# ictnlp/StreamSpeech

Measured on AMD Instinct MI355X. Metric: real-time factor (RTFx = audio seconds / wall seconds) + utterances/sec, offline S2ST fr-en, higher is better.
Workload: dtype f32

## Files before the change

### include/streamspeech_hip.h

```cpp
#ifndef STREAMSPEECH_HIP_H
#define STREAMSPEECH_HIP_H

#include <stddef.h>
#include <stdint.h>

#ifdef __cplusplus
extern "C" {
#endif

#define SS_ABI_VERSION 2

typedef struct ss_model ss_model;
typedef struct ss_vocoder ss_vocoder;
typedef struct ss_scratch ss_scratch;
typedef struct ss_stream_pool ss_stream_pool;

typedef struct ss_config {
  int32_t input_feat, conv_channels, conv_kernel;
  int32_t enc_dim, enc_ffn, enc_heads, enc_layers, dw_kernel;
  int32_t src_vocab, tgt_vocab;
  int32_t mt_layers, dec_dim, dec_ffn, dec_heads;
  int32_t t2u_layers, unit_layers, unit_vocab, ctc_upsample;
  int32_t pad, eos, unk;
  int32_t max_rel_pos;
// ... 308 lines not shown
int ss_batch_cmvn(ss_model* m, void* stream, const float* d_in, int64_t rows, float* d_out);
int ss_batch_encoder_forward(ss_model* m, void* stream, int B, const float* d_fbank, const int32_t* h_T,
                             int attn_chunk, int conv_chunk, float* d_enc_out, int32_t* h_Tp);
int ss_batch_ctc_greedy(ss_model* m, void* stream, int head, int B, const float* d_enc_out,
                        const int32_t* h_Tp, int32_t* d_raw, int32_t* d_tokens, int32_t* d_index,
                        int32_t* d_counts);
int ss_batch_ctc_greedy_scored(ss_model* m, void* stream, int head, int B, const float* d_enc_out,
                               const int32_t* h_Tp, int32_t* d_raw, int32_t* d_tokens, int32_t* d_index,
                               int32_t* d_counts, float* d_lprob, int32_t* d_last, float* d_tok_lprob);
typedef struct ss_ctc_align_result {
  double score;
  double viterbi;
  int32_t status;
  int32_t n_tokens;
} ss_ctc_align_result;
#define SS_CTC_ALIGN_MAX_FRAMES 1500
#define SS_CTC_ALIGN_MAX_LABELS 1500
int ss_batch_ctc_align(ss_model* m, void* stream, int head, int B, const float* d_enc_out, const int32_t* h_Tp,
                       const int32_t* h_targets, const int32_t* h_n_targets, ss_ctc_align_result* d_results, int32_t* d_path,
                       int32_t* d_first, int32_t* d_last, float* d_tok_lprob);
int ss_ctc_align_host(const float* h_logits, int ld, int V, int pad, int B, const int32_t* h_T, const int32_t* h_targets,
                      const int32_t* h_n_targets, ss_ctc_align_result* h_results, int32_t* h_path, int32_t* h_first, int32_t* h_last,
                      float* h_tok_lprob, float* h_frame_lprob);
int ss_batch_mt_greedy(ss_model* m, void* stream, int B, const float* d_enc_out, const int32_t* h_Tp,
                       const int32_t* h_max_len, int min_len, int32_t* h_out_tokens, int out_stride,
                       int32_t* h_n_out, float* d_feats, int feat_rows);
int ss_batch_mt_beam(ss_model* m, void* stream, int B, int beam, const float* d_enc_out, const int32_t* h_Tp,
                     const int32_t* h_max_len, int min_len, float unk_penalty, int normalize, int32_t* h_out_tokens,
                     int out_stride, int32_t* h_n_out, float* h_scores, float* h_pos_scores, float* d_feats, int feat_rows);
int ss_batch_mt_continue(ss_model* m, void* stream, int B, const float* d_enc_out, const int32_t* h_Tp, const int32_t* h_prefix,
                         const int32_t* h_n_prefix, const int32_t* h_max_len, int min_len, int32_t* h_out_tokens, int out_stride,
                         int32_t* h_n_out, float* d_feats, int feat_rows, int32_t* h_n_feats);
int ss_batch_mt_continue_plan(int B, const int32_t* h_Tp, const int32_t* h_prefix, const int32_t* h_n_prefix, const int32_t* h_max_len,
                              int min_len, int out_stride, int feat_rows, int max_tgt_pos, int vocab, int eos, int32_t* h_dims,
                              int32_t* h_tables, int64_t tables_cap, int64_t* h_n_tables);
int ss_batch_mt_beam_continue(ss_model* m, void* stream, int B, int beam, const float* d_enc_out, const int32_t* h_Tp,
                              const int32_t* h_prefix, const int32_t* h_n_prefix, const int32_t* h_max_len, int min_len,
                              float unk_penalty, int normalize, int32_t* h_out_tokens, int out_stride, int32_t* h_n_out,
                              float* h_scores, float* h_pos_scores, float* d_feats, int feat_rows);
int ss_batch_mt_beam_continue_plan(int B, int beam, const int32_t* h_Tp, const int32_t* h_prefix, const int32_t* h_n_prefix,
                                   const int32_t* h_max_len, int min_len, int out_stride, int feat_rows, int max_tgt_pos, int vocab,
                                   int eos, int pad, int32_t* h_dims, int32_t* h_tables, int64_t tables_cap, int64_t* h_n_tables);
typedef struct ss_mt_search_opts {
  int32_t size;
  int32_t no_repeat_ngram;
  float len_penalty;
  float temperature;
} ss_mt_search_opts;
int ss_batch_mt_beam_opts(ss_model* m, void* stream, int B, int beam, const float* d_enc_out, const int32_t* h_Tp,
                          const int32_t* h_max_len, int min_len, float unk_penalty, int normalize, int32_t* h_out_tokens,
                          int out_stride, int32_t* h_n_out, float* h_scores, float* h_pos_scores, float* d_feats, int feat_rows,
                          const ss_mt_search_opts* opts);
int ss_batch_mt_beam_continue_opts(ss_model* m, void* stream, int B, int beam, const float* d_enc_out, const int32_t* h_Tp,
                                   const int32_t* h_prefix, const int32_t* h_n_prefix, const int32_t* h_max_len, int min_len,
                                   float unk_penalty, int normalize, int32_t* h_out_tokens, int out_stride, int32_t* h_n_out,
                                   float* h_scores, float* h_pos_scores, float* d_feats, int feat_rows,
                                   const ss_mt_search_opts* opts);
int ss_batch_mt_beam_continue_plan_opts(int B, int beam, const int32_t* h_Tp, const int32_t* h_prefix, const int32_t* h_n_prefix,
                                        const int32_t* h_max_len, int min_len, int out_stride, int feat_rows, int max_tgt_pos,
                                        int vocab, int eos, int pad, int32_t* h_dims, int32_t* h_tables, int64_t tables_cap,
                                        int64_t* h_n_tables, const ss_mt_search_opts* opts);
typedef struct ss_mt_sample_opts {
  int32_t size;
  int32_t topk;
  float topp;
  int32_t reserved;
  uint64_t seed;
} ss_mt_sample_opts;
int ss_batch_mt_sample(ss_model* m, void* stream, int B, int beam, const float* d_enc_out, const int32_t* h_Tp,
                       const int32_t* h_max_len, int min_len, float unk_penalty, int normalize, int32_t* h_out_tokens, int out_stride,
                       int32_t* h_n_out, float* h_scores, float* h_pos_scores, float* d_feats, int feat_rows,
                       const ss_mt_search_opts* opts, const int64_t* h_keys, const ss_mt_sample_opts* sample);
int ss_batch_mt_sample_continue(ss_model* m, void* stream, int B, int beam, const float* d_enc_out, const int32_t* h_Tp,
                                const int32_t* h_prefix, const int32_t* h_n_prefix, const int32_t* h_max_len, int min_len,
                                float unk_penalty, int normalize, int32_t* h_out_tokens, int out_stride, int32_t* h_n_out,
                                float* h_scores, float* h_pos_scores, float* d_feats, int feat_rows, const ss_mt_search_opts* opts,
                                const int64_t* h_keys, const ss_mt_sample_opts* sample);
int ss_batch_fbank_frames(ss_model* m, void* stream, int B, const float* const* h_pcm, const int32_t* h_first, const int32_t* h_n,
                          float pcm_scale, float* const* h_feat);
int ss_batch_fbank_frames_sr(ss_model* m, void* stream, int B, const float* const* h_pcm, const int32_t* h_n_in, const int32_t* h_up,
                             const int32_t* h_down, const float* const* h_taps, const int32_t* h_half_len, const int32_t* h_first,
                             const int32_t* h_n, float pcm_scale, float* const* h_feat);
int ss_fbank_sr_rows(int64_t n_in, int up, int down, int half_len, int32_t* h_n_rows, int32_t* h_n_final);
int ss_batch_t2u_units(ss_model* m, void* stream, int B, const float* d_feats, int feat_rows,
                       const int32_t* h_n, int t2u_causal, int mask_eos, int32_t* d_raw, int32_t* d_tokens,
                       int32_t* d_counts);
int ss_batch_vocoder_forward(ss_vocoder* v, void* stream, int B, const int32_t* d_codes, const int32_t* h_K,
                             int dur_prediction, const int32_t* d_forced_dur, float* d_wav,
                             int64_t wav_capacity, int32_t* d_dur, int64_t* h_wav_start,
                             int64_t* h_n_samples);
int ss_batch_vocoder_forward_spkr(ss_vocoder* v, void* stream, int B, const int32_t* d_codes, const int32_t* h_K,
                                  int dur_prediction, const int32_t* d_forced_dur, float* d_wav,
                                  int64_t wav_capacity, int32_t* d_dur, int64_t* h_wav_start,
                                  int64_t* h_n_samples, const int32_t* h_spkr );
int ss_batch_t2u_units_pad(ss_model* m, void* stream, int B, const float* d_feats, int feat_rows, const int32_t* h_n,
                           const int32_t* h_n_tail_pad, int t2u_causal, int mask_eos, int32_t* d_raw, int32_t* d_tokens,
                           int32_t* d_counts);
int ss_batch_mt_features(ss_model* m, void* stream, int B, const float* d_enc_out, const int32_t* h_Tp, const int32_t* h_tokens,
                         const int32_t* h_n_tokens, const int32_t* h_n_tail_pad, float* d_feats, int feat_rows);
int ss_batch_mt_attention(ss_model* m, void* stream, int B, const float* d_enc_out, const int32_t* h_Tp, const int32_t* h_tokens,
                          const int32_t* h_n_tokens, const int32_t* h_first, float* d_feats, int feat_rows, float* d_attn,
                          int64_t* h_attn_off, int64_t attn_capacity, int32_t* d_peak, float* d_stat);
int ss_batch_mt_score(ss_model* m, void* stream, int U, const float* d_enc_out, const int32_t* h_Tp, int B, const int32_t* h_src,
                      const int32_t* h_tokens, const int32_t* h_n_tokens, float* d_feats, int feat_rows, float* d_stat,
                      int32_t* d_idx);
int ss_batch_vocoder_tail(ss_vocoder* v, void* stream, int B, const int32_t* d_codes, const int32_t* h_K, const int32_t* h_n_new,
                          const int32_t* h_ctx, const int32_t* h_rf, int dur_prediction, float* d_out, int64_t out_capacity,
                          int32_t* h_win_first, int32_t* h_dur, int64_t* h_out_start, int64_t* h_n_out);
int ss_batch_vocoder_tail_spkr(ss_vocoder* v, void* stream, int B, const int32_t* d_codes, const int32_t* h_K, const int32_t* h_n_new,
                               const int32_t* h_ctx, const int32_t* h_rf, int dur_prediction, float* d_out, int64_t out_capacity,
                               int32_t* h_win_first, int32_t* h_dur, int64_t* h_out_start, int64_t* h_n_out,
                               const int32_t* h_spkr );

int ss_batch_unit_spans(ss_model* m, void* stream, int B, const int32_t* d_raw, const int32_t* h_n, const int32_t* h_K,
                        const int32_t* h_dur_first, const int32_t* h_unit0, const int32_t* d_dur, const int32_t* h_dur,
                        int32_t* h_spans, int32_t* h_K_out);
int ss_unit_spans_host(int B, const int32_t* h_raw, const int32_t* h_n, const int32_t* h_K, const int32_t* h_dur_first,
                       const int32_t* h_unit0, const int32_t* h_dur, int up, int blank, int pad, int bos, int eos, int32_t* h_spans,
                       int32_t* h_K_out);

int ss_prof_enable(int cls_mask);
int ss_prof_enable_hi(int cls_mask);
int ss_prof_reset(void);
int ss_prof_read(int cls, double* h_ms_total, double* h_flops_total, int64_t* h_launches,
                 double* h_bytes_total);
int ss_prof_totals(int cls, double* h_flops_total, double* h_bytes_total, int64_t* h_launches);
int ss_prof_read_issued(int cls, double* h_issued_flops_total);
int ss_prof_shape_log(int on);
int ss_prof_shape_dump(char* buf, int cap);
int ss_prof_num_classes(void);
const char* ss_prof_class_name(int cls);

int ss_model_set_pack_invariant(ss_model* m, int on);
int ss_model_get_pack_invariant(ss_model* m);
int ss_debug_canon(int mode);

int ss_debug_last_logits(ss_model* m, void* stream, float* d_out, int64_t cap_floats, int* h_rows, int* h_cols);

int ss_op_ffn_fused(void* stream, const float* dX, int ldx, float* dY, int ldy, const float* ln_g, const float* ln_b,
                    const float* dW1, const float* db1, const float* dW2, const float* db2, float alpha,
                    const float* ln2_g, const float* ln2_b, int M, int D, int F);
int ss_debug_ffn(int grid, int row_tiles_per_wave, int enable);
int ss_debug_rtlin(int grid, int enable);
int ss_debug_rtlin_kb(int uw, int order);
int ss_debug_rtlin_kb_last(int32_t out[4]);
int ss_debug_conv_c64(int enable);
int ss_debug_conv_c256_rows(int rows);
int ss_debug_conv_c32(int enable);
int ss_debug_conv_c16(int enable);
int64_t ss_debug_enc_step_launches(void);
int ss_op_ln_linear(void* stream, const float* dX, int ldx, const float* ln_g, const float* ln_b, const float* dW,
                    const float* dbias, const float* dR, int ldr, float* dC, int ldc, int M, int N, int K, int act, float alpha,
                    int glu);
int ss_op_ln_linear_ex(void* stream, const float* dX, int ldx, const float* ln_g, const float* ln_b, float* ln_out, const float* dW,
                       const float* dbias, const float* dR, int ldr, float* dC, int ldc, int M, int N, int K, int act, float alpha,
                       int glu, int canon);

int ss_debug_force_tile(int bm, int bn, int ks);
int ss_debug_sk_errors(void);
int ss_debug_attention_split(int v);
int ss_debug_attention_q16(int v);
int ss_debug_enc_step_inject_timeout(ss_model* m);
int ss_debug_scratch_audit(ss_scratch* sc, size_t* booked, size_t* held);
int ss_debug_mt_inject_timeout(ss_model* m);

int ss_op_conv_gemm(void* stream, const float* dA, int lda, const float* dW, const float* dbias,
                    const float* dR, int ldr, const float* dR2, int ldr2, float* dC, int ldc,
                    int M, int N, int Cin, int taps, int dil, int stride, int pad, int in_len,
                    int chunk, int in_act, float in_slope, int act, float alpha, float div, int glu);
typedef struct ss_op_conv_args {
  const float* A; const float* W; const float* bias; const float* R; const float* R2; float* C; float* C2;
  int32_t lda, ldc, ldr, ldr2, ldc2;
  int32_t M, N, Cin, taps, dil, stride, pad, in_len, chunk;
  int32_t in_act; float in_slope;
  int32_t act; float act_slope, alpha, div, c2_slope;
  int32_t glu;
  const int32_t* segs; int32_t nseg, max_seg_out;
  int32_t same_rows;
} ss_op_conv_args;
int ss_op_conv_gemm_ex(void* stream, const ss_op_conv_args* a);
int ss_op_conv_gemm_rows(void* stream, const ss_op_conv_args* a, int m_begin, const int32_t* seg_mb, const float* const* seg_A, int canon);
int ss_op_conv_pair(void* stream, const float* dA, int lda, const float* dW1, const float* db1, const float* dW2, const float* db2,
                    float* dC, int ldc, const float* dR2, int ldr2, float div, float* dC2, int ldc2, float c2_slope, int C, int taps,
                    int dil, int M, int in_len, float slope, const int32_t* d_segs, int nseg);
int ss_op_resblock_fused(void* stream, const float* dX, int ldx, const float* const* dW1, const float* const* dB1,
                         const float* const* dW2, const float* const* dB2, const int32_t* dil, float* dY, int ldy, const float* dR2,
                         int ldr2, float div, int C, int taps, int M, float slope, const int32_t* d_segs, int nseg);
int ss_debug_slab(int grid, long long min_rows);
int ss_op_conv_f16(void* stream, const float* dA, const float* dW, const float* dbias, const float* dR, const float* dR2,
                   float* dC, float* dC2, int M, int C, int taps, int dil, int in_act, float in_slope, int act, float div,
                   const int32_t* d_segs, int nseg);
int ss_op_layernorm(void* stream, const float* dx, int ldx, float* dy, int ldy, const float* dg,
                    const float* db, int M, int D, float eps);
int ss_op_attention(void* stream, const float* dQ, int ldq, const float* dK, int ldk, const float* dV,
                    int ldv, float* dO, int ldo, int Tq, int Tk, int H, float scale, int causal,
                    int chunk, const float* dP, int ldp, const float* du, const float* dv);
typedef struct ss_op_attn_args {
  const float* Q; const float* K; const float* V; float* O;
  int32_t ldq, ldk, ldv, ldo;
  int32_t Tq, Tk, H;
  float scale;
  int32_t causal, chunk, q0, k_mask_tail;
  const float* P; int32_t ldp;
  const float* bias_u; const float* bias_v;
  const int32_t* segs; int32_t nseg, max_q, p_tmax;
  const int32_t* seg_tail;
  int32_t no_decode_kernel;
  const int32_t* anc; int32_t anc_ld, anc_slots;
  int32_t use_split;
} ss_op_attn_args;
int ss_op_attention_ex(void* stream, const ss_op_attn_args* a);
typedef struct ss_op_attn_probs_args {
  const float* Q; const float* K;
  int32_t ldq, ldk, H;
  float scale;
  const int32_t* segs; int32_t nseg;
  const int32_t* q_first; const int32_t* row_off; const int64_t* p_off;
  float* P; int32_t* peak; float* stat;
  int32_t max_rows;
} ss_op_attn_probs_args;
int ss_op_attention_probs(void* stream, const ss_op_attn_probs_args* a);
typedef struct ss_op_pool_attn_args {
  const float* Qs; float* cache; float* O;
  int32_t ld, ldo, slot_rows;
  const float* P; int32_t ldp, p_tmax;
  const float* bias_u; const float* bias_v;
  const int32_t* sess; const int32_t* qt_pre;
  int32_t nsess, qtiles, H;
// ... 92 lines not shown
```

### streamspeech_amd/csrc/batch.hip

```cpp
#include <cstring>
#include "model_internal.hpp"
#include "ctc_align.hpp"

extern "C" int ss_batch_fbank_cmvn(ss_model* m, void* stream, int B, const float* d_pcm, const int64_t* h_pcm_start,
                                   const int32_t* h_n_samples, float pcm_scale, float* d_feat, int32_t* h_T) {
  if (!m || B <= 0 || !d_pcm || !d_feat || !h_pcm_start || !h_n_samples || !h_T) return SS_ERR_ARG;
  int64_t rows = 0;
  for (int b = 0; b < B; ++b) {
    if (h_n_samples[b] < 0 || h_pcm_start[b] < 0 || h_pcm_start[b] > (int64_t)0x7fffffff) return SS_ERR_ARG;
    rows += ss_fbank_num_frames(h_n_samples[b]);
  }
  if (rows > (int64_t)0x7fffffff) return SS_ERR_ARG;
  hipStream_t s = (hipStream_t)stream;
  std::vector<int> segs(3 * (size_t)B);
  int row = 0;
  for (int b = 0; b < B; ++b) {
    const int T = ss_fbank_num_frames(h_n_samples[b]);
    h_T[b] = T;
    segs[3 * (size_t)b] = (int)h_pcm_start[b]; segs[3 * (size_t)b + 1] = T; segs[3 * (size_t)b + 2] = row;
    row += T;
  }
  if (row == 0) return SS_OK;
  RET(m->sc->seg_buf.ensure(segs.size() * sizeof(int)));
  const int* dt = (const int*)m->sc->seg_buf.p;
  RET(upload(s, (int*)m->sc->seg_buf.p, segs));
  constexpr int kSlice = 65535;
  for (int b0 = 0; b0 < B; b0 += kSlice) {
    const int nb = std::min(kSlice, B - b0);
    int mx = 0;
    for (int b = b0; b < b0 + nb; ++b) mx = std::max(mx, segs[3 * (size_t)b + 1]);
    RET(launch_fbank_cmvn_batch(d_pcm, pcm_scale, m->fe_window, m->fe_melw, m->fe_mean, m->fe_std, d_feat, dt + 3 * (size_t)b0, nb,
                                mx, s));
  }
  return SS_OK;
}

extern "C" int ss_batch_cmvn(ss_model* m, void* stream, const float* d_in, int64_t rows, float* d_out) {
  if (!m || rows < 0 || (rows > 0 && (!d_in || !d_out))) return SS_ERR_ARG;
  return launch_cmvn_rows(d_in, rows, m->fe_mean, m->fe_std, d_out, (hipStream_t)stream);
}

extern "C" int ss_batch_encoder_forward(ss_model* m, void* stream, int B, const float* d_fbank, const int32_t* h_T,
                                        int attn_chunk, int conv_chunk, float* d_enc_out, int32_t* h_Tp) {
  if (!m || B <= 0) return SS_ERR_ARG;
  SkScope sk_scope(m->sc->skws);
  CanonScope canon_scope(m->pack_invariant ? CANON_SEQ : CANON_NONE);
  const bool canon = m->pack_invariant && !debug_tile_forced();
  hipStream_t s = (hipStream_t)stream;
  const ss_config& c = m->cfg;
  const int d = c.enc_dim, f = c.enc_ffn, k = c.conv_kernel, Ld = c.enc_layers * d;
  std::vector<int> T1(B), T2(B);
  for (int b = 0; b < B; ++b) {
    if (h_T[b] <= 0) return SS_ERR_ARG;
    T1[b] = conv_out_len(h_T[b], k, 2); T2[b] = conv_out_len(T1[b], k, 2);
    if (T2[b] <= 0 || T2[b] > c.max_rel_pos) return SS_ERR_CAPACITY;
    h_Tp[b] = T2[b];
  }
  const Offsets o0 = prefix(h_T, B), o1 = prefix(T1.data(), B), o2 = prefix(T2.data(), B);
  const int M1 = o1.total, M2 = o2.total;
  const int cchunk = conv_chunk_cfg(conv_chunk);
  const int achunk = attn_chunk_cfg(attn_chunk);

  std::vector<int> tab(14 * B);
  int* t0 = tab.data(); int* t1 = t0 + 4 * B; int* ta = t1 + 4 * B; int* tr = ta + 4 * B;
  for (int b = 0; b < B; ++b) {
    t0[4 * b] = o1.off[b]; t0[4 * b + 1] = T1[b]; t0[4 * b + 2] = o0.off[b]; t0[4 * b + 3] = h_T[b];
    t1[4 * b] = o2.off[b]; t1[4 * b + 1] = T2[b]; t1[4 * b + 2] = o1.off[b]; t1[4 * b + 3] = T1[b];
    ta[4 * b] = o2.off[b]; ta[4 * b + 1] = T2[b]; ta[4 * b + 2] = o2.off[b]; ta[4 * b + 3] = T2[b];
    tr[2 * b] = o2.off[b]; tr[2 * b + 1] = T2[b];
  }
  RET(m->sc->seg_buf.ensure(tab.size() * sizeof(int)));
  int* dt = (int*)m->sc->seg_buf.p;
  RET(upload(s, dt, tab));
  const int *d0 = dt, *d1 = dt + 4 * B, *da = dt + 8 * B, *dr = dt + 12 * B;

  const size_t n_h1 = (size_t)M1 * (c.conv_channels / 2), n_x = (size_t)M2 * d, n_f = (size_t)M2 * f,
               n_qkv = (size_t)M2 * 3 * d;
  RET(m->sc->ws.ensure((n_h1 + 3 * n_x + n_f + n_qkv) * sizeof(float)));
  float* h1 = m->sc->ws.f();
  float* x = d_enc_out;
  float* h = h1 + n_h1;
  float* g = h + n_x;
  float* g2 = g + n_x;
  float* ff = g2 + n_x;
  float* qkv = ff + n_f;
  GemmArgs a, b;
  subsampler_args(m, d_fbank, h1, g, a, b);
  a.chunk = cchunk; a.segs = d0; a.nseg = B; a.max_seg_out = o1.mx; a.M = M1; a.in_len = o0.total;
  b.chunk = cchunk; b.segs = d1; b.nseg = B; b.max_seg_out = o2.mx; b.M = M2; b.in_len = M1;
  RET(launch_conv_gemm(a, s));
  RET(launch_conv_gemm(b, s));
  RET(linear(s, g, d, M2, m->enc_linear, d, d, x, d));
  for (int l = 0; l < c.enc_layers; ++l) {
    const EncLayer& e = m->enc[l];
    const bool fuse_ffn = (canon || (disp().ffn_fusion && M2 >= disp().ffn_min_rows)) && ffn_fused_eligible(d, f, ACT_SILU, M2, d, d, canon) &&
                          e.ffn1_w1.b && e.ffn1_w2.b && e.ffn2_w1.b && e.ffn2_w2.b;
    if (canon && !fuse_ffn) return SS_ERR_ARG;
    auto attention = [&] {
      AttnArgs at;
      at.Q = qkv; at.K = qkv + d; at.V = qkv + 2 * d; at.ldq = at.ldk = at.ldv = 3 * d;
      at.O = h; at.ldo = d; at.H = c.enc_heads; at.scale = 0.125f; at.chunk = achunk;
      at.P = m->pos_proj + (size_t)l * d; at.ldp = Ld; at.p_tmax = c.max_rel_pos; at.bias_u = e.u; at.bias_v = e.v;
      at.segs = da; at.nseg = B; at.max_q = o2.mx;
      return launch_attention(at, s);
    };
    auto dwconv = [&] {
      return launch_dwconv_bn_silu(g, d, g2, d, e.dw_wt, c.dw_kernel, e.bn_mean, e.bn_var, e.bn_g, e.bn_b, 1e-5f, o2.mx, d, cchunk, s,
                                   dr, B);
    };
    RET(enc_layer_ex(s, c, e, x, M2, h, ff, qkv, g, g2, fuse_ffn, canon, attention, dwconv));
  }
  return SS_OK;
}

// ... 103 lines not shown
  int Lmax = 0;
  for (int b = 0; b < B; ++b) {
    if (h_Tp[b] <= 0 || h_max_len[b] < 0) return SS_ERR_ARG;
    Lmax = std::max(Lmax, h_max_len[b]);
  }
  const int Lcap = Lmax + 2;
  if (Lcap > feat_rows || Lcap + 2 > c.max_tgt_pos || out_stride < Lmax + 1) return SS_ERR_CAPACITY;
  const Offsets oe = prefix(h_Tp, B);
  RET(m->sc->mt_cross.ensure((size_t)c.mt_layers * oe.total * 2 * D * sizeof(float)));
  RET(mt_cross_kv(m, s, d_enc_out, oe.total));
  RET(m->sc->bmt_self.ensure((size_t)c.mt_layers * B * Lcap * 3 * D * sizeof(float)));
  RET(m->sc->mt_ws.ensure(MtRowsWs::floats(B, D, F, V) * sizeof(float)));
  const MtRowsWs w(m->sc->mt_ws.f(), B, D, F);
  const size_t n_tok = (size_t)(Lcap + 1) * B;
  RET(m->sc->seg_buf.ensure((n_tok + B + 4 * B + (size_t)Lcap * 4 * B) * sizeof(int)));
  int* tok = (int*)m->sc->seg_buf.p;
  int* d_maxlen = tok + n_tok;
  int* d_cross = d_maxlen + B;
  int* d_self = d_cross + 4 * B;
  {
    std::vector<int> t0(B, c.eos), ml(h_max_len, h_max_len + B), cs(4 * B), ss((size_t)Lcap * 4 * B);
    for (int b = 0; b < B; ++b) { cs[4 * b] = b; cs[4 * b + 1] = 1; cs[4 * b + 2] = oe.off[b]; cs[4 * b + 3] = h_Tp[b]; }
    for (int st = 0; st < Lcap; ++st)
      for (int b = 0; b < B; ++b) {
        int* e = &ss[((size_t)st * B + b) * 4];
        e[0] = b; e[1] = 1; e[2] = b * Lcap; e[3] = st + 1;
      }
    RET(upload(s, tok, t0)); RET(upload(s, d_maxlen, ml)); RET(upload(s, d_cross, cs)); RET(upload(s, d_self, ss));
  }
  std::vector<int> host_tok(n_tok, c.pad);
  std::vector<int> eos_at(B, -1);
  int checked = 1;
  int step = 0;
  constexpr int kCheck = 4;
  CanonScope decode_scope(m->pack_invariant ? CANON_SMALLM : CANON_NONE);
  while (true) {
    MtRowsStep a;
    a.rows = B; a.cache_ld = Lcap; a.ci = step; a.tok = tok + (size_t)step * B;
    a.self_segs = d_self + (size_t)step * 4 * B; a.cross_segs = d_cross; a.n_enc = oe.total;
    a.states = d_feats + (size_t)step * D; a.states_ld = feat_rows * D;
    RET(mt_decode_rows(m, s, w, a));
    RET(launch_masked_argmax(w.logits, V, B, V, c.pad, step < min_len ? c.eos : -1, -1, -1, tok + (size_t)(step + 1) * B, s,
                             d_maxlen, step, c.eos));
    ++step;
    const bool last = step > Lmax;
    if (last || step % kCheck == 0) {
      SS_HIP_CHECK(hipMemcpyAsync(host_tok.data() + (size_t)checked * B, tok + (size_t)checked * B,
                                  (size_t)(step + 1 - checked) * B * sizeof(int), hipMemcpyDeviceToHost, s));
      SS_HIP_CHECK(hipStreamSynchronize(s));
      bool all_done = true;
      for (int b = 0; b < B; ++b) {
        for (int r = checked; r <= step && eos_at[b] < 0; ++r)
          if (host_tok[(size_t)r * B + b] == c.eos) eos_at[b] = r;
        if (eos_at[b] < 0) all_done = false;
      }
      checked = step + 1;
      if (all_done || last) break;
    }
  }
  for (int b = 0; b < B; ++b) {
    const int end = eos_at[b] >= 0 ? eos_at[b] : step;
    h_n_out[b] = end;
    for (int r = 1; r <= end; ++r) h_out_tokens[(size_t)b * out_stride + (r - 1)] = host_tok[(size_t)r * B + b];
  }
  return SS_OK;
}

static int batch_t2u(ss_model* m, void* stream, int B, const float* d_feats, int feat_rows, const int32_t* h_n, const int32_t* h_pad,
                     int t2u_causal, int mask_eos, int32_t* d_raw, int32_t* d_tokens, int32_t* d_counts) {
  if (!m || B <= 0 || !h_n) return SS_ERR_ARG;
  SkScope sk_scope(m->sc->skws);
  CanonScope canon_scope(m->pack_invariant ? CANON_SEQ : CANON_NONE);
  hipStream_t s = (hipStream_t)stream;
  const ss_config& c = m->cfg;
  const int D = c.dec_dim, F = c.dec_ffn, V = c.unit_vocab, H = c.dec_heads, up = c.ctc_upsample;
  for (int b = 0; b < B; ++b)
    if (h_n[b] <= 0) return SS_ERR_ARG;
  if (h_pad)
    for (int b = 0; b < B; ++b)
      if (h_pad[b] < 0 || h_pad[b] >= h_n[b]) return SS_ERR_ARG;
  const Offsets on = prefix(h_n, B);
  const int Nn = on.total, U = Nn * up;
  const size_t nx = (size_t)U * D;
  RET(m->sc->ws.ensure((3 * nx + (size_t)U * 3 * D + (size_t)U * F + (size_t)Nn * 2 * D + (size_t)Nn * D +
                    (size_t)U * V + (size_t)U) * sizeof(float)));
  float* x = m->sc->ws.f();
  float* h = x + nx;
  float* q2 = h + nx;
  float* selfbuf = q2 + nx;
  float* ff = selfbuf + (size_t)U * 3 * D;
  float* crosskv = ff + (size_t)U * F;
  float* t2u_out = crosskv + (size_t)Nn * 2 * D;
  float* logits = t2u_out + (size_t)Nn * D;
  int32_t* idx_scratch = reinterpret_cast<int32_t*>(logits + (size_t)U * V);
  std::vector<int> tab(14 * B + Nn + (h_pad ? 3 * B : 0));
  for (int b = 0; b < B; ++b) {
    const int o = on.off[b], n = h_n[b];
    for (int r = 0; r < n; ++r) tab[14 * B + o + r] = b * feat_rows + r;
    int* a = &tab[4 * b]; a[0] = o; a[1] = n; a[2] = o; a[3] = n;
    int* u = &tab[4 * B + 4 * b]; u[0] = o * up; u[1] = n * up; u[2] = o * up; u[3] = n * up;
    int* x2 = &tab[8 * B + 4 * b]; x2[0] = o * up; x2[1] = n * up; x2[2] = o; x2[3] = n;
    tab[12 * B + 2 * b] = o * up; tab[12 * B + 2 * b + 1] = n * up;
    if (h_pad) {
      int* k = &tab[14 * B + Nn];
      k[b] = h_pad[b]; k[B + b] = h_pad[b] * up; k[2 * B + b] = h_pad[b];
    }
  }
  RET(m->sc->seg_buf.ensure(tab.size() * sizeof(int)));
  int* dt = (int*)m->sc->seg_buf.p;
  RET(upload(s, dt, tab));
  const int* tail = h_pad ? dt + 14 * B + Nn : nullptr;
  for (int b = 0; b < B; ++b)
    if (h_n[b] > feat_rows) return SS_ERR_CAPACITY;
  RET(launch_gather_rows(dt + 14 * B, d_feats, D, x, Nn, s, B * feat_rows));
  for (int l = 0; l < c.t2u_layers; ++l) {
    AttnArgs at;
    at.Q = selfbuf; at.ldq = 3 * D; at.K = selfbuf + D; at.V = selfbuf + 2 * D; at.ldk = at.ldv = 3 * D;
    at.O = h; at.ldo = D; at.H = H; at.scale = 1.f; at.causal = t2u_causal ? 1 : 0;
    at.segs = dt; at.nseg = B; at.max_q = on.mx;
    at.no_decode_kernel = m->pack_invariant;
    at.seg_tail = tail;
    RET(dec_layer_ex(s, c, m->t2u[l], x, Nn, selfbuf, 3 * D, at, nullptr, h, q2, ff));
  }
  RET(launch_layernorm(x, D, t2u_out, D, m->t2u_ln.g, m->t2u_ln.b, Nn, D, 1e-5f, s));
  RET(launch_upsample_add_pos(t2u_out, Nn, up, m->unit_pos_row, (float)c.pad, x, D, s));
  for (int l = 0; l < c.unit_layers; ++l) {
    RET(linear(s, t2u_out, D, Nn, m->unit[l].cross_kv, 2 * D, D, crosskv, 2 * D));
    AttnArgs at;
    at.Q = selfbuf; at.ldq = 3 * D; at.K = selfbuf + D; at.V = selfbuf + 2 * D; at.ldk = at.ldv = 3 * D;
    at.O = h; at.ldo = D; at.H = H; at.scale = 1.f; at.causal = 1;
    at.segs = dt + 4 * B; at.nseg = B; at.max_q = on.mx * up; at.no_decode_kernel = m->pack_invariant;
    AttnArgs ac;
    ac.Q = q2; ac.ldq = D; ac.K = crosskv; ac.V = crosskv + D; ac.ldk = ac.ldv = 2 * D;
    ac.O = h; ac.ldo = D; ac.H = H; ac.scale = 1.f; ac.segs = dt + 8 * B; ac.nseg = B; ac.max_q = on.mx * up;
    ac.no_decode_kernel = m->pack_invariant;
    if (tail) { at.seg_tail = tail + B; ac.seg_tail = tail + 2 * B; }
    RET(dec_layer_ex(s, c, m->unit[l], x, U, selfbuf, 3 * D, at, &ac, h, q2, ff));
  }
  RET(launch_layernorm(x, D, h, D, m->unit_ln.g, m->unit_ln.b, U, D, 1e-5f, s));
  RET(linear(s, h, D, U, m->unit_out, V, D, logits, V));
  m->sc->dbg_logits = logits; m->sc->dbg_rows = U; m->sc->dbg_cols = V;
  RET(launch_masked_argmax(logits, V, U, V, c.pad, c.unk, mask_eos ? c.eos : -1, -1, d_raw, s));
  return launch_ctc_collapse(d_raw, 0, V - 1, c.pad, d_tokens, idx_scratch, d_counts, s, dt + 12 * B, B);
}

extern "C" int ss_batch_t2u_units(ss_model* m, void* stream, int B, const float* d_feats, int feat_rows,
                                  const int32_t* h_n, int t2u_causal, int mask_eos, int32_t* d_raw, int32_t* d_tokens,
                                  int32_t* d_counts) {
  return batch_t2u(m, stream, B, d_feats, feat_rows, h_n, nullptr, t2u_causal, mask_eos, d_raw, d_tokens, d_counts);
}

extern "C" int ss_batch_t2u_units_pad(ss_model* m, void* stream, int B, const float* d_feats, int feat_rows, const int32_t* h_n,
                                      const int32_t* h_n_tail_pad, int t2u_causal, int mask_eos, int32_t* d_raw, int32_t* d_tokens,
                                      int32_t* d_counts) {
  if (!h_n_tail_pad) return SS_ERR_ARG;
  return batch_t2u(m, stream, B, d_feats, feat_rows, h_n, h_n_tail_pad, t2u_causal, mask_eos, d_raw, d_tokens, d_counts);
}

struct McPlan {
  int S = 0, Tn = 0, Lcap = 0, Tr = 0, Np = 0, np_max = 0;
  std::vector<int> head;
};
static int mt_continue_plan(int B, const int32_t* h_Tp, const int32_t* h_prefix, const int32_t* h_n_prefix, const int32_t* h_max_len,
                            int min_len, int out_stride, int feat_rows, int max_tgt_pos, int vocab, int eos, McPlan& P) {
  if (B <= 0 || B > 256 || !h_Tp || !h_n_prefix || !h_max_len) return SS_ERR_ARG;
  int S = 0, Tn = 0, Np = 0, np_max = 0;
  for (int b = 0; b < B; ++b) {
    const int st = h_n_prefix[b];
    if (h_Tp[b] <= 0 || st < 0 || h_max_len[b] < st) return SS_ERR_ARG;
    if (st > 0 && !h_prefix) return SS_ERR_ARG;
    S = std::max(S, st);
    Tn = std::max(Tn, h_max_len[b] - st);
    Np += st + 1;
    np_max = std::max(np_max, st + 1);
  }
  {
    int o = 0;
    for (int b = 0; b < B; ++b) {
      for (int i = 0; i < h_n_prefix[b]; ++i)
        if (h_prefix[o + i] < 0 || h_prefix[o + i] >= vocab) return SS_ERR_ARG;
      o += h_n_prefix[b];
    }
  }
  for (int b = 0; b < B; ++b)
    if (h_max_len[b] + 1 > feat_rows || h_max_len[b] - h_n_prefix[b] + 1 > out_stride || h_max_len[b] + 3 > max_tgt_pos)
      return SS_ERR_CAPACITY;
  const int Lcap = S + 1 + Tn, Tr = std::max(Tn, 1);
  const Offsets oe = prefix(h_Tp, B);
  std::vector<int> seg_len(B);
  for (int b = 0; b < B; ++b) seg_len[b] = h_n_prefix[b] + 1;
  const Offsets op = prefix(seg_len.data(), B);
  const size_t np = (size_t)Np;
  P.S = S; P.Tn = Tn; P.Lcap = Lcap; P.Tr = Tr; P.Np = Np; P.np_max = np_max;
  P.head.assign(15 * (size_t)B + (size_t)Tr * 4 * B + 4 * np + B, 0);
  int* ml = P.head.data(); int* mn = ml + B; int* rp = mn + B; int* cs = rp + B; int* ps = cs + 4 * B; int* pc = ps + 4 * B;
  int* ls = pc + 4 * B; int* pt = ls + (size_t)Tr * 4 * B; int* pp = pt + np; int* pk = pp + np; int* pf = pk + np; int* pl = pf + np;
  int o = 0;
  for (int b = 0; b < B; ++b) {
    const int st = h_n_prefix[b], sh = S - st, r0 = op.off[b];
    ml[b] = h_max_len[b] + sh; mn[b] = min_len + sh; rp[b] = -sh;
    cs[4 * b] = b; cs[4 * b + 1] = 1; cs[4 * b + 2] = oe.off[b]; cs[4 * b + 3] = h_Tp[b];
    ps[4 * b] = r0; ps[4 * b + 1] = st + 1; ps[4 * b + 2] = r0; ps[4 * b + 3] = st + 1;
    pc[4 * b] = r0; pc[4 * b + 1] = st + 1; pc[4 * b + 2] = oe.off[b]; pc[4 * b + 3] = h_Tp[b];
    for (int t = 0; t < Tr; ++t) {
      int* e = &ls[((size_t)t * B + b) * 4];
      e[0] = b; e[1] = 1; e[2] = b * Lcap + sh; e[3] = st + 2 + t;
    }
    for (int p = 0; p <= st; ++p) {
      pt[r0 + p] = p == 0 ? eos : h_prefix[o + p - 1];
      pp[r0 + p] = p;
      pk[r0 + p] = b * Lcap + sh + p;
      pf[r0 + p] = b * feat_rows + p;
    }
    pl[b] = r0 + st;
    o += st;
  }
  return SS_OK;
}

// ... 237 lines not shown
  hipStream_t s = (hipStream_t)stream;
  int* dt = (int*)m->sc->seg_buf.p;
  RET(upload(s, dt, tab));
  const int *d_self = dt, *d_cross = dt + 4 * B, *d_tail = dt + 8 * B, *d_tok = dt + 9 * B, *d_pos = d_tok + np, *d_frow = d_pos + np;
  RET(mt_cross_kv(m, s, d_enc_out, oe.total));
  const float* pfo = nullptr;
  RET(mt_prefix_pass(m, s, B, Np, op.mx, oe.total, d_tok, d_pos, d_self, d_cross, d_tail, nullptr, 0, &pfo));
  if (d_feats) RET(launch_scatter_rows(d_frow, pfo, D, d_feats, D, D, Np, B * feat_rows, s));
  if (so) {
    float* logits = m->sc->ws.f() + np * (7 * D + F);
    const int* d_tgt = dt + n_base;
    Lin proj{m->mt_emb, nullptr};
    for (int r0 = 0; r0 < Np; r0 += kMtScoreChunk) {
      const int rows = std::min(kMtScoreChunk, Np - r0);
      RET(linear(s, pfo + (size_t)r0 * D, D, rows, proj, V, D, logits, V));
      RET(launch_mt_token_scores(logits, V, rows, V, d_tgt + r0, so->d_stat + 2 * (size_t)r0, so->d_idx + 2 * (size_t)r0, s));
    }
    return SS_OK;
  }
  if (!ao) return SS_OK;
  AttnProbsArgs ap;
  ap.Q = m->sc->ws.f() + 2 * np * D; ap.ldq = D;
  ap.K = m->sc->mt_cross.f() + (size_t)(c.mt_layers - 1) * oe.total * 2 * D; ap.ldk = 2 * D;
  ap.H = c.dec_heads; ap.scale = 1.f;
  ap.segs = d_cross; ap.nseg = B;
  ap.q_first = dt + n_base; ap.row_off = dt + n_base + B;
  ap.p_off = reinterpret_cast<const long long*>(dt + n_off);
  ap.P = ao->d_attn; ap.peak = ao->d_peak; ap.stat = ao->d_stat; ap.max_rows = max_rows;
  return launch_attention_probs(ap, s);
}

extern "C" int ss_batch_mt_features(ss_model* m, void* stream, int B, const float* d_enc_out, const int32_t* h_Tp,
                                    const int32_t* h_tokens, const int32_t* h_n_tokens, const int32_t* h_n_tail_pad, float* d_feats,
                                    int feat_rows) {
  if (!h_n_tail_pad || !d_feats) return SS_ERR_ARG;
  return batch_mt_features(m, stream, B, d_enc_out, h_Tp, h_tokens, h_n_tokens, h_n_tail_pad, d_feats, feat_rows, nullptr);
}

extern "C" int ss_batch_mt_attention(ss_model* m, void* stream, int B, const float* d_enc_out, const int32_t* h_Tp,
                                     const int32_t* h_tokens, const int32_t* h_n_tokens, const int32_t* h_first, float* d_feats,
                                     int feat_rows, float* d_attn, int64_t* h_attn_off, int64_t attn_capacity, int32_t* d_peak,
                                     float* d_stat) {
  if (!d_peak || !d_stat || attn_capacity < 0) return SS_ERR_ARG;
  MtAttnOut ao;
  ao.h_first = h_first; ao.d_attn = d_attn; ao.h_attn_off = h_attn_off; ao.attn_capacity = attn_capacity;
  ao.d_peak = d_peak; ao.d_stat = d_stat;
  return batch_mt_features(m, stream, B, d_enc_out, h_Tp, h_tokens, h_n_tokens, nullptr, d_feats, feat_rows, &ao);
}

extern "C" int ss_batch_mt_score(ss_model* m, void* stream, int U, const float* d_enc_out, const int32_t* h_Tp, int B,
                                 const int32_t* h_src, const int32_t* h_tokens, const int32_t* h_n_tokens, float* d_feats,
                                 int feat_rows, float* d_stat, int32_t* d_idx) {
  if (!d_stat || !d_idx) return SS_ERR_ARG;
  MtScoreOut so;
  so.U = U; so.h_src = h_src; so.d_stat = d_stat; so.d_idx = d_idx;
  return batch_mt_features(m, stream, B, d_enc_out, h_Tp, h_tokens, h_n_tokens, nullptr, d_feats, feat_rows, nullptr, &so);
}

extern "C" int ss_batch_fbank_frames(ss_model* m, void* stream, int B, const float* const* h_pcm, const int32_t* h_first,
                                     const int32_t* h_n, float pcm_scale, float* const* h_feat) {
  if (!m || B <= 0 || B > 65535 || !h_pcm || !h_first || !h_n || !h_feat) return SS_ERR_ARG;
  constexpr int kShift = 160;
  int mx = 0;
  for (int b = 0; b < B; ++b) {
    if (h_first[b] < 0 || h_n[b] < 0 || ((int64_t)h_first[b] + (int64_t)h_n[b]) * kShift > (int64_t)0x7fffffff) return SS_ERR_ARG;
    if (h_n[b] > 0 && (!h_pcm[b] || !h_feat[b])) return SS_ERR_ARG;
    mx = std::max(mx, h_n[b]);
  }
  if (mx == 0) return SS_OK;
  hipStream_t s = (hipStream_t)stream;
  const size_t n_seg = (3 * (size_t)B + 1) & ~(size_t)1;
  std::vector<int> tab(n_seg + 4 * (size_t)B, 0);
  int64_t* ptrs = reinterpret_cast<int64_t*>(tab.data() + n_seg);
  for (int b = 0; b < B; ++b) {
    tab[3 * b] = h_first[b] * kShift; tab[3 * b + 1] = h_n[b]; tab[3 * b + 2] = 0;
    ptrs[b] = (int64_t)(uintptr_t)h_pcm[b];
    ptrs[B + b] = (int64_t)(uintptr_t)h_feat[b];
  }
  RET(m->sc->seg_buf.ensure(tab.size() * sizeof(int)));
  int* dt = (int*)m->sc->seg_buf.p;
  RET(upload(s, dt, tab));
  const float* const* d_pcm = reinterpret_cast<const float* const*>(dt + n_seg);
  float* const* d_feat = reinterpret_cast<float* const*>(dt + n_seg + 2 * (size_t)B);
  return launch_fbank_cmvn_ptrs(d_pcm, d_feat, pcm_scale, m->fe_window, m->fe_melw, m->fe_mean, m->fe_std, dt, B, mx, s);
}

extern "C" int ss_batch_fbank_frames_sr(ss_model* m, void* stream, int B, const float* const* h_pcm, const int32_t* h_n_in,
                                        const int32_t* h_up, const int32_t* h_down, const float* const* h_taps,
                                        const int32_t* h_half_len, const int32_t* h_first, const int32_t* h_n, float pcm_scale,
                                        float* const* h_feat) {
  if (!m || B <= 0 || B > 65535 || !h_pcm || !h_n_in || !h_up || !h_down || !h_taps || !h_half_len || !h_first || !h_n || !h_feat)
    return SS_ERR_ARG;
  static_assert(sizeof(FbankSrSeg) % sizeof(int) == 0, "the segment table is uploaded as ints");
  constexpr size_t kSegInts = sizeof(FbankSrSeg) / sizeof(int);
  std::vector<int> tab(kSegInts * (size_t)B, 0);
  int mx = 0, max_taps = 0;
  for (int b = 0; b < B; ++b) {
    if (h_first[b] < 0 || h_n[b] < 0) return SS_ERR_ARG;
    FbankSrSeg sg{};
    if (h_n[b] > 0) {
      int rows = 0;
      RET(fbank_sr_rows(h_n_in[b], h_up[b], h_down[b], h_half_len[b], &rows, nullptr));
      if ((int64_t)h_first[b] + (int64_t)h_n[b] > (int64_t)rows) return SS_ERR_ARG;
      const bool pass = h_up[b] == h_down[b];
      if (!h_pcm[b] || !h_feat[b] || (!pass && !h_taps[b])) return SS_ERR_ARG;
      sg.pcm = h_pcm[b]; sg.taps = h_taps[b]; sg.feat = h_feat[b];
      sg.n_in = h_n_in[b]; sg.up = h_up[b]; sg.down = h_down[b]; sg.half = h_half_len[b]; sg.first = h_first[b]; sg.n_rows = h_n[b];
      mx = std::max(mx, h_n[b]);
      if (!pass) max_taps = std::max(max_taps, 2 * h_half_len[b] + 1);
    }
    std::memcpy(tab.data() + kSegInts * (size_t)b, &sg, sizeof(sg));
  }
  if (mx == 0) return SS_OK;
  hipStream_t s = (hipStream_t)stream;
  RET(m->sc->seg_buf.ensure(tab.size() * sizeof(int)));
  int* dt = (int*)m->sc->seg_buf.p;
  RET(upload(s, dt, tab));
  return launch_fbank_cmvn_sr(reinterpret_cast<const FbankSrSeg*>(dt), B, mx, max_taps, pcm_scale, m->fe_window, m->fe_melw,
                              m->fe_mean, m->fe_std, s);
}

extern "C" int ss_fbank_sr_rows(int64_t n_in, int up, int down, int half_len, int32_t* h_n_rows, int32_t* h_n_final) {
  int rows = 0, fin = 0;
  RET(fbank_sr_rows(n_in, up, down, half_len, &rows, &fin));
  if (h_n_rows) *h_n_rows = rows;
  if (h_n_final) *h_n_final = fin;
  return SS_OK;
}
```

### streamspeech_amd/csrc/debug_ops.hip

```cpp
#include "model_internal.hpp"
#include "ctc_align.hpp"

static int op_bind_wino(GemmArgs& a, void* stream) {
  static thread_local std::map<hipStream_t, DevBuf> wino_tmps;
  DevBuf& wino_tmp = wino_tmps[(hipStream_t)stream];
  const int N = a.N, Cin = a.Cin, taps = a.taps;
  if ((conv_c64w_enabled() && N == 64 && Cin == 64 && taps >= 3 && conv_c64_eligible(a)) ||
      (conv_c128w_enabled() && N == 128 && Cin == 128 && taps >= 3 && a.same_rows && !a.glu) ||
      (conv_c256w_enabled() && N == 256 && Cin == 256 && taps >= 3 && a.same_rows && !a.glu) ||
      (conv_c32w_enabled() && N == 32 && Cin == 32 && taps >= 3 && conv_c32_eligible(a))) {
    RET(wino_tmp.ensure((size_t)N * ((taps + 2) / 3) * 4 * N * sizeof(float)));
    RET(launch_wino_pack(a.W, wino_tmp.f(), N, taps, (hipStream_t)stream));
    a.Wwino = wino_tmp.f();
  }
  return SS_OK;
}

extern "C" int ss_op_conv_gemm(void* stream, const float* dA, int lda, const float* dW, const float* dbias,
                               const float* dR, int ldr, const float* dR2, int ldr2, float* dC, int ldc, int M,
                               int N, int Cin, int taps, int dil, int stride, int pad, int in_len, int chunk,
                               int in_act, float in_slope, int act, float alpha, float div, int glu) {
  GemmArgs a;
  a.A = dA; a.lda = lda; a.W = dW; a.bias = dbias; a.R = dR; a.ldr = ldr; a.R2 = dR2; a.ldr2 = ldr2; a.C = dC; a.ldc = ldc;
  a.M = M; a.N = N; a.Cin = Cin; a.taps = taps; a.dil = dil; a.stride = stride; a.pad = pad; a.in_len = in_len;
// ... 69 lines not shown

extern "C" int ss_debug_last_logits(ss_model* m, void* stream, float* d_out, int64_t cap_floats, int* h_rows, int* h_cols) {
  if (!m || !h_rows || !h_cols) return SS_ERR_ARG;
  *h_rows = m->sc->dbg_rows; *h_cols = m->sc->dbg_cols;
  if (!d_out) return SS_OK;
  if (!m->sc->dbg_logits || cap_floats < (int64_t)m->sc->dbg_rows * m->sc->dbg_cols) return SS_ERR_CAPACITY;
  SS_HIP_CHECK(hipMemcpyAsync(d_out, m->sc->dbg_logits, (size_t)m->sc->dbg_rows * m->sc->dbg_cols * sizeof(float), hipMemcpyDeviceToDevice,
                              (hipStream_t)stream));
  return SS_OK;
}

extern "C" int ss_op_ffn_fused(void* stream, const float* dX, int ldx, float* dY, int ldy, const float* ln_g, const float* ln_b,
                               const float* dW1, const float* db1, const float* dW2, const float* db2, float alpha,
                               const float* ln2_g, const float* ln2_b, int M, int D, int F) {
  return launch_ffn_fused(dX, ldx, dY, ldy, ln_g, ln_b, dW1, db1, dW2, db2, alpha, ln2_g, ln2_b, M, D, F, (hipStream_t)stream,
                          canon_mode() == CANON_SEQ);
}
extern "C" int ss_debug_canon(int mode) {
  if (mode < 0 || mode > 2) return SS_ERR_ARG;
  canon_debug_set(mode);
  return SS_OK;
}
extern "C" int ss_op_ln_linear(void* stream, const float* dX, int ldx, const float* ln_g, const float* ln_b, const float* dW,
                               const float* dbias, const float* dR, int ldr, float* dC, int ldc, int M, int N, int K, int act,
                               float alpha, int glu) {
  GemmArgs a;
  a.A = dX; a.lda = ldx; a.W = dW; a.bias = dbias; a.R = dR; a.ldr = ldr; a.C = dC; a.ldc = ldc;
  a.M = M; a.N = N; a.Cin = K; a.in_len = M; a.act = act; a.alpha = alpha; a.glu = glu; a.same_rows = 1;
  a.ln_g = ln_g; a.ln_b = ln_b;
  return launch_conv_gemm(a, (hipStream_t)stream);
}
extern "C" int ss_op_ln_linear_ex(void* stream, const float* dX, int ldx, const float* ln_g, const float* ln_b, float* ln_out,
                                  const float* dW, const float* dbias, const float* dR, int ldr, float* dC, int ldc, int M, int N, int K,
                                  int act, float alpha, int glu, int canon) {
  if (canon < 0 || canon > 2 || (ln_g == nullptr) != (ln_b == nullptr) || (ln_out && !ln_g)) return SS_ERR_ARG;
  GemmArgs a;
  a.A = dX; a.lda = ldx; a.W = dW; a.bias = dbias; a.R = dR; a.ldr = ldr; a.C = dC; a.ldc = ldc;
  a.M = M; a.N = N; a.Cin = K; a.in_len = M; a.act = act; a.alpha = alpha; a.glu = glu; a.same_rows = 1;
  a.ln_g = ln_g; a.ln_b = ln_b; a.ln_out = ln_out; a.canon = canon;
  return launch_conv_gemm(a, (hipStream_t)stream);
}
extern "C" int ss_debug_conv_c64(int enable) {
  if (enable == 4 || enable == 5) { conv_c64w_debug(enable == 5); return SS_OK; }
  if (enable == 6 || enable == 7) { conv_c128w_debug(enable == 7); return SS_OK; }
  if (enable == 8 || enable == 9) { conv_c256w_debug(enable == 9); return SS_OK; }
  conv_c64_debug(enable);
  return SS_OK;
}
extern "C" int ss_debug_conv_c256_rows(int rows) { return conv_c256w_rows_debug(rows); }
extern "C" int ss_debug_conv_c32(int enable) {
  if (enable == 4 || enable == 5) { conv_c32w_debug(enable == 5); return SS_OK; }
  conv_c32_debug(enable);
  return SS_OK;
}
extern "C" int ss_debug_conv_c16(int enable) { conv_c16_debug(enable); return SS_OK; }
extern "C" int64_t ss_debug_enc_step_launches(void) { return (int64_t)enc_step_launch_count(); }
extern "C" int ss_debug_scratch_audit(ss_scratch* sc, size_t* booked, size_t* held) {
  if (!sc || !booked || !held) return SS_ERR_ARG;
  size_t sum = 0;
  bool foreign = false;
  for (DevBuf* b : sc->all()) {
    sum += b->bytes;
    if (b->acct != &sc->acct) foreign = true;
  }
  *booked = sc->acct.used;
  *held = sum;
  return foreign ? SS_ERR_ARG : SS_OK;
}
extern "C" int ss_debug_rtlin(int grid, int enable) {
  if (grid < 0) return SS_ERR_ARG;
  rtlin_debug(grid, enable);
  return SS_OK;
}
extern "C" int ss_debug_rtlin_kb(int uw, int order) {
  if (!(uw == 0 || uw == 1 || uw == 2 || uw == 4) || order < -1 || order > 2) return SS_ERR_ARG;
  rtlin_kb_debug(uw, order);
  return SS_OK;
}
extern "C" int ss_debug_rtlin_kb_last(int32_t out[4]) {
  if (!out) return SS_ERR_ARG;
  int v[4];
  rtlin_kb_last(v);
  for (int i = 0; i < 4; ++i) out[i] = v[i];
  return SS_OK;
}
extern "C" int ss_debug_ffn(int grid, int row_tiles_per_wave, int enable) {
  if (grid < 0 || row_tiles_per_wave < -1 || row_tiles_per_wave > 4) return SS_ERR_ARG;
  ffn_fused_debug_grid(grid);
  ffn_fused_debug_rows(row_tiles_per_wave);
  if (enable >= 0) dispatch_edit([enable](Dispatch& d) { d.ffn_fusion = enable ? 1 : 0; });
  return SS_OK;
}

extern "C" int ss_op_layernorm(void* stream, const float* dx, int ldx, float* dy, int ldy, const float* dg,
                               const float* db, int M, int D, float eps) {
  return launch_layernorm(dx, ldx, dy, ldy, dg, db, M, D, eps, (hipStream_t)stream);
}

extern "C" int ss_op_masked_argmax(void* stream, const float* logits, int ld, int M, int N, int mask0, int mask1, int mask2, int force,
                                   int32_t* ids, const int32_t* row_max_len, int step, int force_id, const int32_t* row_min_len,
                                   int ban_id) {
  return launch_masked_argmax(logits, ld, M, N, mask0, mask1, mask2, force, ids, (hipStream_t)stream, row_max_len, step, force_id,
                              row_min_len, ban_id);
}
extern "C" int ss_op_ctc_collapse(void* stream, const int32_t* raw, int T, int blank, int pad, int32_t* tokens, int32_t* index,
                                  int32_t* count, const int32_t* segs, int nseg) {
  return launch_ctc_collapse(raw, T, blank, pad, tokens, index, count, (hipStream_t)stream, segs, nseg);
}
extern "C" int ss_op_masked_argmax_lprob(void* stream, const float* logits, int ld, int M, int N, int mask0, int mask1, int mask2,
                                         int32_t* ids, float* lprob) {
  return launch_masked_argmax_lprob(logits, ld, M, N, mask0, mask1, mask2, ids, lprob, (hipStream_t)stream);
}
static int g_mt_score_form = 0;
extern "C" int ss_debug_mt_score_form(int v) { g_mt_score_form = v ? 1 : 0; return SS_OK; }
extern "C" int ss_op_mt_token_scores(void* stream, const float* d_logits, int ld, int rows, int V, const int32_t* d_target,
                                     float* d_stat, int32_t* d_idx) {
  return launch_mt_token_scores(d_logits, ld, rows, V, d_target, d_stat, d_idx, (hipStream_t)stream, g_mt_score_form);
}
extern "C" int ss_op_ctc_collapse_spans(void* stream, const int32_t* raw, const float* lprob, int T, int blank, int pad, int32_t* tokens,
                                        int32_t* index, int32_t* last, float* tok_lprob, int32_t* count, const int32_t* segs, int nseg) {
  return launch_ctc_collapse_spans(raw, lprob, T, blank, pad, tokens, index, last, tok_lprob, count, (hipStream_t)stream, segs, nseg);
}
extern "C" int ss_op_ctc_align(void* stream, const float* d_logits, int ld, int V, int pad, int B, const int32_t* h_T,
                               const int32_t* h_targets, const int32_t* h_n_targets, ss_ctc_align_result* d_results, int32_t* d_path,
                               int32_t* d_first, int32_t* d_last, float* d_tok_lprob, float* d_frame_lprob) {
  if (!d_logits || ld < V || !d_results) return SS_ERR_ARG;
  CtcAlignPlan plan;
  RET(ctc_align_plan(V, pad, B, h_T, h_targets, h_n_targets, plan));
  if (plan.labels > 0 && (!d_first || !d_last || !d_tok_lprob)) return SS_ERR_ARG;
  static thread_local std::map<hipStream_t, std::pair<DevBuf, DevBuf>> tmps;
  auto& tmp = tmps[(hipStream_t)stream];
  RET(tmp.first.ensure(ctc_align_table_bytes(plan)));
  RET(tmp.second.ensure(plan.work_bytes()));
  return launch_ctc_align(d_logits, ld, V, plan, h_targets, tmp.first.p, tmp.second.p, d_results, d_path, d_first, d_last, d_tok_lprob,
                          d_frame_lprob, (hipStream_t)stream);
}
extern "C" int ss_op_dur_predict(void* stream, const float* logdur, const int32_t* forced, int K, int32_t* dur, int32_t* cum,
                                 const int32_t* segs, int nseg) {
  return launch_dur_predict(logdur, forced, K, dur, cum, (hipStream_t)stream, segs, nseg);
}
extern "C" int ss_op_repeat_rows(void* stream, const float* emb, const int32_t* cum, int K, int D, float* out, int F,
                                 const int32_t* segs, int nseg) {
  return launch_repeat_rows(emb, cum, K, D, out, F, (hipStream_t)stream, segs, nseg);
}
extern "C" int ss_op_embed_tokens(void* stream, const int32_t* tok, const float* emb, const float* pos_table, float scale, int pos0,
                                  float* out, int n, int D, int pos_stride, int pad_id, int vocab) {
  return launch_embed_tokens(tok, emb, pos_table, scale, pos0, out, n, D, (hipStream_t)stream, pos_stride, pad_id, vocab);
}
extern "C" int ss_op_embed_tokens_rows(void* stream, const int32_t* tok, const float* emb, const float* pos_table, int pos_rows,
                                       float scale, int pos0, const int32_t* row_pos, float* out, int n, int D, int pad_id, int vocab) {
  return launch_embed_tokens_rows(tok, emb, pos_table, pos_rows, scale, pos0, row_pos, out, n, D, (hipStream_t)stream, pad_id, vocab);
}
extern "C" int ss_op_upsample_add_pos(void* stream, const float* src, int n, int up, const float* pos_row, float pad_value, float* out,
                                      int D) {
  return launch_upsample_add_pos(src, n, up, pos_row, pad_value, out, D, (hipStream_t)stream);
}
extern "C" int ss_op_gather_rows(void* stream, const int32_t* idx, const float* table, int D, float* out, int n, int rows) {
  return launch_gather_rows(idx, table, D, out, n, (hipStream_t)stream, rows);
}
extern "C" int ss_op_scatter_rows(void* stream, const int32_t* dst_row, const float* src, int lds, float* dst, int ldd, int D, int n,
                                  int dst_rows) {
  return launch_scatter_rows(dst_row, src, lds, dst, ldd, D, n, dst_rows, (hipStream_t)stream);
}
extern "C" int ss_op_conv_post_tanh(void* stream, const float* x, int T, int C, const float* w, const float* bias, float slope,
                                    float* wav, const int32_t* segs, int nseg) {
  return launch_conv_post_tanh(x, T, C, w, bias, slope, wav, (hipStream_t)stream, segs, nseg);
// ... 117 lines not shown
```

### streamspeech_amd/csrc/dispatch.hip

```cpp
#include "gemm.hpp"

#include <atomic>
#include <cstdlib>
#include <map>
#include <mutex>
#include <utility>
#include <vector>

namespace ss {

namespace {
std::mutex g_disp_mu;
std::atomic<unsigned> g_disp_gen{1};
Dispatch env_defaults() {
  Dispatch d;
  auto I = [](const char* k, int dflt) { const char* e = getenv(k); return e ? atoi(e) : dflt; };
  auto L = [](const char* k, long long dflt) { const char* e = getenv(k); return e ? atoll(e) : dflt; };
  d.attn_split = I("SS_ATTN_NO_SPLIT", 0) ? -1 : 0; d.attn_q16 = I("SS_ATTN_Q16", d.attn_q16);
  d.c16_off = I("SS_NO_CONV_C16", 0) ? 1 : 0; d.c32_off = I("SS_NO_CONV_C32", 0) ? 1 : 0; d.c64_off = I("SS_NO_CONV_C64", 0) ? 1 : 0;
  d.c16_min_rows = L("SS_CONV_C16_MIN_ROWS", d.c16_min_rows); d.c32_min_rows = L("SS_CONV_C32_MIN_ROWS", d.c32_min_rows);
  d.c64_min_rows = L("SS_CONV_C64_MIN_ROWS", d.c64_min_rows);
  d.c64w_on = I("SS_CONV_C64_WINOGRAD", 1); d.c128w_on = I("SS_CONV_C128_WINOGRAD", 1); d.c256w_on = I("SS_CONV_C256_WINOGRAD", 1);
  d.c32w_on = I("SS_CONV_C32_WINOGRAD", 1); d.c64w_min_k = I("SS_CONV_C64_WINOGRAD_MIN_K", 3);
  d.c128w_min_rows = L("SS_CONV_C128_MIN_ROWS", d.c128w_min_rows); d.c256w_min_rows = L("SS_CONV_C256_MIN_ROWS", d.c256w_min_rows);
  if (const int r = I("SS_CONV_C256_ROWS", d.c256w_rows); r == 128 || r == 256) d.c256w_rows = r;
  if (getenv("SS_FFN_WM")) { d.ffn_wm = I("SS_FFN_WM", 3); d.ffn_wm_forced = 1; d.ffn_wm_env = d.ffn_wm; }
  d.ffn_fusion = I("SS_NO_FFN_FUSION", 0) ? 0 : 1; d.ffn_min_rows = I("SS_FFN_MIN_ROWS", d.ffn_min_rows);
  if (getenv("SS_SK_MIN_GFLOP")) d.sk_min_flops = 1e9 * atof(getenv("SS_SK_MIN_GFLOP"));
  d.no_resblock_fusion = I("SS_NO_RESBLOCK_FUSION", 0); d.no_pair_fusion = I("SS_NO_PAIR_FUSION", 0);
  d.rt_off = I("SS_NO_RTLIN", 0) ? 1 : 0; d.rt_min_rows = I("SS_RTLIN_MIN_ROWS", d.rt_min_rows); d.rt_min_units = L("SS_RTLIN_MIN_UNITS", d.rt_min_units);
  d.rt_kb_min_units = L("SS_RTLIN_KB_MIN_UNITS", d.rt_kb_min_units); d.rt_kb_uw = I("SS_RTLIN_KB_UW", d.rt_kb_uw); d.rt_kb_xmap = I("SS_RTLIN_KB_XMAP", d.rt_kb_xmap);
  d.smallm_max_rows = I("SS_SMALLM_MAX_ROWS", d.smallm_max_rows); d.sk_min_units = L("SS_SK_MIN_UNITS", d.sk_min_units);
  d.no_sk2 = I("SS_NO_SK2", 0) ? 1 : 0; d.sk2_min_k64 = I("SS_SK2_MINK64", d.sk2_min_k64); d.sk2_spare_cus = I("SS_SK2_SPARE_CUS", 0);
  d.rt_wg_per_cu = I("SS_RTLIN_WG_PER_CU", 0); d.c32_min_k = I("SS_CONV_C32_MIN_K", d.c32_min_k); d.c16_min_k = I("SS_CONV_C16_MIN_K", d.c16_min_k);
  return d;
}
Dispatch& process_settings() { static Dispatch d = env_defaults(); return d; }
thread_local const Dispatch* t_disp = nullptr;
thread_local CtxDispatch t_disp_own;
}
void dispatch_edit(const std::function<void(Dispatch&)>& fn) {
  std::lock_guard<std::mutex> lk(g_disp_mu);
  fn(process_settings());
  g_disp_gen.fetch_add(1, std::memory_order_release);
}
void slab_debug(int grid, long long min_rows) {
  const Dispatch dflt = env_defaults();
  dispatch_edit([=](Dispatch& d) {
    d.slab_grid_cap = grid > 0 ? grid : 0;
    const bool set = min_rows >= 0;
    d.c16_min_rows = set ? min_rows : dflt.c16_min_rows; d.c32_min_rows = set ? min_rows : dflt.c32_min_rows;
    d.c64_min_rows = set ? min_rows : dflt.c64_min_rows;
    d.c128w_min_rows = set ? min_rows : dflt.c128w_min_rows; d.c256w_min_rows = set ? min_rows : dflt.c256w_min_rows;
  });
}
int conv_c256w_rows_debug(int rows) {
  if (rows != 0 && rows != 128 && rows != 256) return SS_ERR_ARG;
  const int dflt = env_defaults().c256w_rows;
  dispatch_edit([=](Dispatch& d) { d.c256w_rows = rows ? rows : dflt; });
  return SS_OK;
}
const Dispatch* CtxDispatch::refresh() {
  const unsigned now = g_disp_gen.load(std::memory_order_acquire);
  if (gen != now) {
    std::lock_guard<std::mutex> lk(g_disp_mu);
    d = process_settings();
    gen = g_disp_gen.load(std::memory_order_relaxed);
  }
  return &d;
}
const Dispatch& disp() { return t_disp ? *t_disp : *t_disp_own.refresh(); }
DispatchScope::DispatchScope(const Dispatch* d) : prev(t_disp) { t_disp = d; }
DispatchScope::~DispatchScope() { t_disp = prev; }

void debug_force_tile(int bm, int bn, int ks) {
  dispatch_edit([=](Dispatch& d) { d.force_bm = bm; d.force_bn = bn; d.force_ks = ks; d.sk_groups = (bm == 1 && bn == 8); });
}
bool debug_tile_forced() { return disp().force_bm != 0; }

static thread_local int t_canon = CANON_NONE;
CanonScope::CanonScope(int mode) : prev(t_canon) { t_canon = mode; }
CanonScope::~CanonScope() { t_canon = prev; }
int canon_mode() { return t_canon; }
void canon_debug_set(int mode) { t_canon = mode; }

constexpr size_t SKW_SYNC_BYTES = (16 + 1024) * sizeof(unsigned) + 256;
static std::mutex g_skw_mu;
static std::vector<SkWorkspace*> g_skw_live;
static std::map<std::pair<int, hipStream_t>, SkWorkspace*> g_skw_fallback;
static thread_local SkWorkspace* t_skw = nullptr;

SkWorkspace* sk_workspace_new() {
  SkWorkspace* w = new SkWorkspace();
  std::lock_guard<std::mutex> lk(g_skw_mu);
  g_skw_live.push_back(w);
  return w;
}
void sk_workspace_free(SkWorkspace* w) {
  if (!w) return;
  {
    std::lock_guard<std::mutex> lk(g_skw_mu);
    for (size_t i = 0; i < g_skw_live.size(); ++i)
      if (g_skw_live[i] == w) { g_skw_live.erase(g_skw_live.begin() + i); break; }
  }
  if (w->ws) (void)hipFree(w->ws);
  if (w->sync1) (void)hipFree(w->sync1);
  if (w->sync2) (void)hipFree(w->sync2);
  if (w->sync3) (void)hipFree(w->sync3);
  if (w->dbg) (void)hipFree(w->dbg);
  delete w;
}
SkScope::SkScope(SkWorkspace* w) : prev(t_skw), prev_disp(t_disp) { t_skw = w; t_disp = w ? w->disp.refresh() : nullptr; }
SkScope::~SkScope() { t_skw = prev; t_disp = prev_disp; }

int sk_workspace_acquire(hipStream_t stream, SkWorkspace** out) {
  *out = nullptr;
  int dev = 0;
// ... 58 lines not shown
```

### streamspeech_amd/csrc/dispatch.hpp

```cpp
#pragma once
#include <functional>

namespace ss {

struct Dispatch {
  int attn_no_mfma = 0;
  int attn_q16 = 1;
  int attn_split = 0;
  int c16_off = 0, c32_off = 0, c64_off = 0;
  long long c16_min_rows = 131072, c32_min_rows = 65536, c64_min_rows = 32768;
  int c64w_on = 1, c128w_on = 1, c256w_on = 1, c32w_on = 1;
  int c64w_min_k = 3;
  long long c128w_min_rows = 65536, c256w_min_rows = 32768;
  int c256w_rows = 128;
  int c32_min_k = 7, c16_min_k = 11;
  int slab_grid_cap = 0;
  int sk_groups = 0;
  int sk2_spare_cus = 0;
  int ffn_force_g = 0;
  int ffn_wm = 3, ffn_wm_forced = 0;
  int ffn_wm_env = 0;
  int ffn_fusion = 1;
  int ffn_min_rows = 1000;
  int force_bm = 0, force_bn = 0, force_ks = 0;
  double sk_min_flops = 4e9;
  int smallm_max_rows = 192;
  long long sk_min_units = 12 * 512;
  int no_sk2 = 0;
  int sk2_min_k64 = 192;
  int no_resblock_fusion = 0, no_pair_fusion = 0;
  int rt_off = 0, rt_min_rows = 193, rt_force_g = 0;
  long long rt_min_units = 4000;
  int rt_wg_per_cu = 0;
  long long rt_kb_min_units = 256;
  int rt_kb_xmap = 1;
  int rt_kb_uw = 0;
  int rt_kb_order = 1;
};

const Dispatch& disp();
void dispatch_edit(const std::function<void(Dispatch&)>& fn);

struct CtxDispatch {
  Dispatch d;
  unsigned gen = 0xffffffffu;
  const Dispatch* refresh();
};
struct DispatchScope {
  explicit DispatchScope(const Dispatch* d);
  ~DispatchScope();
  const Dispatch* prev;
};

}
```

### streamspeech_amd/csrc/elementwise.hip

```cpp
#include "elementwise.hpp"

namespace ss {

template <int PER_LANE>
__global__ __launch_bounds__(256) void layernorm_kernel(const float* __restrict__ x, int ldx, float* y,
                                                        int ldy, const float* __restrict__ gamma,
                                                        const float* __restrict__ beta, int M, float eps) {
  constexpr int D = PER_LANE * 64;
  const int lane = threadIdx.x & 63;
  const int row = blockIdx.x * 4 + (threadIdx.x >> 6);
  if (row >= M) return;
  const float* xr = x + (size_t)row * ldx;
  float v[PER_LANE];
  float s = 0.f;
#pragma unroll
  for (int i = 0; i < PER_LANE; ++i) { v[i] = xr[lane + 64 * i]; s += v[i]; }
  const float mean = wave_sum(s) / (float)D;
  float q = 0.f;
#pragma unroll
  for (int i = 0; i < PER_LANE; ++i) { const float d = v[i] - mean; q += d * d; }
  const float rstd = 1.0f / sqrtf(wave_sum(q) / (float)D + eps);
  float* yr = y + (size_t)row * ldy;
#pragma unroll
  for (int i = 0; i < PER_LANE; ++i) {
// ... 62 lines not shown
  const float mean = bn_mean[c], rstd = 1.0f / sqrtf(bn_var[c] + bn_eps), gam = bn_gamma[c], bet = bn_beta[c];
  constexpr int NR = DW_TT / 4, NV = NR + DW_KMAX - 1;
  float sv[NV];
#pragma unroll
  for (int i = 0; i < NV; ++i) sv[i] = slab[(rg * NR + i) * DW_TC + cl];
#pragma unroll
  for (int u = 0; u < NR; ++u) {
    const int t = t0 + rg * NR + u;
    int lim = T;
    if (chunk > 0) { const int cl_end = (t / chunk + 1) * chunk; if (cl_end < lim) lim = cl_end; }
    const int jmax = min(K, lim - (t - half));
    float acc = 0.f;
#pragma unroll
    for (int j = 0; j < DW_KMAX; ++j) {
      const float a2 = fmaf(w[j], sv[u + j], acc);
      acc = (j < jmax) ? a2 : acc;
    }
    const float v = (acc - mean) * rstd * gam + bet;
    if (t < T) y[(size_t)t * ldy + c] = v / (1.0f + expf(-v));
  }
}

int launch_dwconv_bn_silu(const float* x, int ldx, float* y, int ldy, const float* wt, int K,
                          const float* bn_mean, const float* bn_var, const float* bn_gamma,
                          const float* bn_beta, float bn_eps, int T, int C, int chunk, hipStream_t stream,
                          const int* segs, int nseg, int t_begin) {
  if (T - t_begin <= 0) return SS_OK;
  if (K > DW_KMAX || (K & 1) == 0 || t_begin < 0) return SS_ERR_ARG;
  dim3 grid(cdiv(C, DW_TC), cdiv(T - t_begin, DW_TT), nseg > 0 ? nseg : 1);
  hipLaunchKernelGGL(dwconv_bn_silu_kernel, grid, dim3(256), 0, stream, x, ldx, y, ldy, wt, K, bn_mean,
                     bn_var, bn_gamma, bn_beta, bn_eps, T, C, chunk, nseg > 0 ? segs : nullptr, t_begin);
  SS_LAUNCH_CHECK();
  return SS_OK;
}

__global__ void embed_tokens_kernel(const int* __restrict__ tok, const float* __restrict__ emb,
                                    const float* __restrict__ pos_table, float scale, int pos0, float* out,
                                    int n, int D, int pos_stride, int pad_id, int vocab, const int* __restrict__ row_pos,
                                    int pos_rows) {
  const int i = blockIdx.y;
  const int c = blockIdx.x * 256 + threadIdx.x;
  if (c >= D) return;
  int tk = tok[i];
  if ((unsigned)tk >= (unsigned)vocab) tk = 0;
  int pos = (tk == pad_id) ? pad_id : pos0 + (row_pos ? row_pos[i] : i * pos_stride);
  if (row_pos && (unsigned)pos >= (unsigned)pos_rows) pos = pos_rows - 1;
  out[(size_t)i * D + c] = scale * emb[(size_t)tk * D + c] + pos_table[(size_t)pos * D + c];
}

int launch_embed_tokens(const int* tok, const float* emb, const float* pos_table, float scale, int pos0,
                        float* out, int n, int D, hipStream_t stream, int pos_stride, int pad_id, int vocab) {
  if (n <= 0) return SS_OK;
  hipLaunchKernelGGL(embed_tokens_kernel, dim3(cdiv(D, 256), n), dim3(256), 0, stream, tok, emb, pos_table,
                     scale, pos0, out, n, D, pos_stride, pad_id, vocab, (const int*)nullptr, 0);
  SS_LAUNCH_CHECK();
  return SS_OK;
}

int launch_embed_tokens_rows(const int* tok, const float* emb, const float* pos_table, int pos_rows, float scale, int pos0,
                             const int* row_pos, float* out, int n, int D, hipStream_t stream, int pad_id, int vocab) {
  if (n <= 0) return SS_OK;
  if (pos_rows <= 0) return SS_ERR_ARG;
  hipLaunchKernelGGL(embed_tokens_kernel, dim3(cdiv(D, 256), n), dim3(256), 0, stream, tok, emb, pos_table,
                     scale, pos0, out, n, D, 0, pad_id, vocab, row_pos, pos_rows);
  SS_LAUNCH_CHECK();
  return SS_OK;
}

__global__ void upsample_add_pos_kernel(const float* __restrict__ src, int up, const float* __restrict__ pos_row,
                                        float pad_value, float* out, int D) {
  const int u = blockIdx.y;
  const int c = blockIdx.x * 256 + threadIdx.x;
  if (c >= D) return;
  const float* s = src + (size_t)(u / up) * D;
  const float add = (s[0] != pad_value) ? pos_row[c] : 0.f;
  out[(size_t)u * D + c] = s[c] + add;
}

int launch_upsample_add_pos(const float* src, int n, int up, const float* pos_row, float pad_value,
                            float* out, int D, hipStream_t stream) {
  if (n <= 0) return SS_OK;
  hipLaunchKernelGGL(upsample_add_pos_kernel, dim3(cdiv(D, 256), n * up), dim3(256), 0, stream, src, up,
                     pos_row, pad_value, out, D);
  SS_LAUNCH_CHECK();
  return SS_OK;
}

__global__ void gather_rows_kernel(const int* __restrict__ idx, const float* __restrict__ table, int D,
                                   float* out, int rows) {
  const int i = blockIdx.y;
  const int c = blockIdx.x * 256 + threadIdx.x;
  if (c >= D) return;
  int r = idx[i];
  if ((unsigned)r >= (unsigned)rows) r = 0;
  out[(size_t)i * D + c] = table[(size_t)r * D + c];
}

int launch_gather_rows(const int* idx, const float* table, int D, float* out, int n, hipStream_t stream, int rows) {
  if (n <= 0) return SS_OK;
  hipLaunchKernelGGL(gather_rows_kernel, dim3(cdiv(D, 256), n), dim3(256), 0, stream, idx, table, D, out, rows);
  SS_LAUNCH_CHECK();
  return SS_OK;
}

__global__ void scatter_rows_kernel(const int* __restrict__ dst_row, const float* __restrict__ src, int lds, float* dst, int ldd,
                                    int D, int dst_rows) {
  const int i = blockIdx.y;
  const int c = blockIdx.x * 256 + threadIdx.x;
  const int r = dst_row[i];
  if (c >= D || (unsigned)r >= (unsigned)dst_rows) return;
  dst[(size_t)r * ldd + c] = src[(size_t)i * lds + c];
}

int launch_scatter_rows(const int* dst_row, const float* src, int lds, float* dst, int ldd, int D, int n, int dst_rows,
                        hipStream_t stream) {
  if (n <= 0) return SS_OK;
  hipLaunchKernelGGL(scatter_rows_kernel, dim3(cdiv(D, 256), n), dim3(256), 0, stream, dst_row, src, lds, dst, ldd, D, dst_rows);
  SS_LAUNCH_CHECK();
  return SS_OK;
}

__global__ __launch_bounds__(256) void masked_argmax_kernel(const float* __restrict__ logits, int ld, int M, int N,
                                                            int mask0, int mask1, int mask2, int force, int* ids,
                                                            const int* __restrict__ row_max_len, int step, int force_id,
                                                            const int* __restrict__ row_min_len, int ban_id) {
  __shared__ float sb[4];
  __shared__ int si[4];
  const int t = threadIdx.x, lane = t & 63, wave = t >> 6;
  const int row = blockIdx.x;
  if (row_max_len && step >= row_max_len[row]) force = force_id;
  if (row_min_len && step < row_min_len[row]) mask1 = ban_id;
  if (force >= 0) { if (t == 0) ids[row] = force; return; }
  const float* r = logits + (size_t)row * ld;
  float best = -INFINITY;
  int bi = 0x7fffffff;
  for (int n = t; n < N; n += 256) {
    if (n == mask0 || n == mask1 || n == mask2) continue;
    float v = r[n];
    if (v != v) v = -INFINITY;
    if (bi == 0x7fffffff || v > best) { best = v; bi = n; }
  }
#pragma unroll
  for (int o = 32; o > 0; o >>= 1) {
    const float ob = __shfl_xor(best, o, 64);
    const int oi = __shfl_xor(bi, o, 64);
    if (oi != 0x7fffffff && (bi == 0x7fffffff || ob > best || (ob == best && oi < bi))) { best = ob; bi = oi; }
  }
  if (lane == 0) { sb[wave] = best; si[wave] = bi; }
  __syncthreads();
  if (t == 0) {
    for (int w = 1; w < 4; ++w) {
      const float ob = sb[w]; const int oi = si[w];
      if (oi != 0x7fffffff && (bi == 0x7fffffff || ob > best || (ob == best && oi < bi))) { best = ob; bi = oi; }
    }
    ids[row] = bi;
  }
}

int launch_masked_argmax(const float* logits, int ld, int M, int N, int mask0, int mask1, int mask2,
                         int force, int* ids, hipStream_t stream, const int* row_max_len, int step, int force_id,
                         const int* row_min_len, int ban_id) {
  if (M <= 0) return SS_OK;
  hipLaunchKernelGGL(masked_argmax_kernel, dim3(M), dim3(256), 0, stream, logits, ld, M, N, mask0,
                     mask1, mask2, force, ids, row_max_len, step, force_id, row_min_len, ban_id);
  SS_LAUNCH_CHECK();
  return SS_OK;
// ... 300 lines not shown
```

### streamspeech_amd/csrc/elementwise.hpp

```cpp
#pragma once
#include "common.hpp"

struct ss_ctc_align_result;

namespace ss {

int launch_layernorm(const float* x, int ldx, float* y, int ldy, const float* gamma, const float* beta,
                     int M, int D, float eps, hipStream_t stream);

int launch_dwconv_bn_silu(const float* x, int ldx, float* y, int ldy, const float* wt, int K,
                          const float* bn_mean, const float* bn_var, const float* bn_gamma,
                          const float* bn_beta, float bn_eps, int T, int C, int chunk, hipStream_t stream,
                          const int* segs = nullptr, int nseg = 0,
                          int t_begin = 0);

int launch_embed_tokens(const int* tok, const float* emb, const float* pos_table, float scale, int pos0,
                        float* out, int n, int D, hipStream_t stream, int pos_stride, int pad_id, int vocab);
int launch_embed_tokens_rows(const int* tok, const float* emb, const float* pos_table, int pos_rows, float scale, int pos0,
                             const int* row_pos, float* out, int n, int D, hipStream_t stream, int pad_id, int vocab);

int launch_upsample_add_pos(const float* src, int n, int up, const float* pos_row, float pad_value,
                            float* out, int D, hipStream_t stream);

int launch_masked_argmax(const float* logits, int ld, int M, int N, int mask0, int mask1, int mask2,
                         int force, int* ids, hipStream_t stream, const int* row_max_len = nullptr, int step = 0,
                         int force_id = -1,
                         const int* row_min_len = nullptr, int ban_id = -1);

int launch_log_softmax(const float* logits, int ld, int M, int N, int mask0, int mask1, int as_probs, float* out, int ldo,
                       hipStream_t stream);
int launch_row_max_logprob(const float* logits, int ld, int M, int N, int mask0, int mask1, int mask2, float* out,
                           hipStream_t stream);

int launch_ctc_collapse(const int* raw, int T, int blank, int pad, int* tokens, int* index, int* count,
                        hipStream_t stream, const int* segs = nullptr, int nseg = 0);

int launch_masked_argmax_lprob(const float* logits, int ld, int M, int N, int mask0, int mask1, int mask2, int* ids, float* lprob,
                               hipStream_t stream);
int launch_ctc_collapse_spans(const int* raw, const float* lprob, int T, int blank, int pad, int* tokens, int* index, int* last,
                              float* tok_lprob, int* count, hipStream_t stream, const int* segs = nullptr, int nseg = 0);

constexpr int MT_SCORE_MAX_ROWS = 16777215;
constexpr int MT_SCORE_MAX_REG_N = 8192;
int launch_mt_token_scores(const float* logits, int ld, int M, int N, const int* target, float* stat, int* idx, hipStream_t stream,
                           int form = 0);

struct CtcAlignPlan;
size_t ctc_align_table_bytes(const CtcAlignPlan& p);
int launch_ctc_align(const float* logits, int ld, int V, const CtcAlignPlan& p, const int32_t* h_targets, void* d_table, void* d_work,
                     ss_ctc_align_result* results, int* path, int* first, int* last, float* tok_lprob, float* frame_lprob,
                     hipStream_t stream);

int launch_gather_rows(const int* idx, const float* table, int D, float* out, int n, hipStream_t stream, int rows);
int launch_scatter_rows(const int* dst_row, const float* src, int lds, float* dst, int ldd, int D, int n, int dst_rows,
                        hipStream_t stream);

int launch_dur_predict(const float* logdur, const int* forced, int K, int* dur, int* cum, hipStream_t stream,
                       const int* segs = nullptr, int nseg = 0);

int launch_repeat_rows(const float* emb, const int* cum, int K, int D, float* out, int F, hipStream_t stream,
                       const int* segs = nullptr, int nseg = 0);

int launch_conv_post_tanh(const float* x, int T, int C, const float* w, const float* bias, float slope,
                          float* wav, hipStream_t stream, const int* segs = nullptr, int nseg = 0);
int launch_conv_post_tanh_crop(const float* x, int C, const float* w, const float* bias, float slope, float* wav, const int* segs,
                               int nseg, int max_keep, hipStream_t stream);

int launch_spkr_pre_add(const float* x, float* y, int ld, int C0, const float* table, const int* spkr, int spkr0, const int* segs,
                        int nseg, int max_seg_out, int M, int act, float slope, hipStream_t stream);

}
```

### streamspeech_amd/csrc/fbank.hip

```cpp
#include "fbank.hpp"

namespace ss {

constexpr int WIN = 400, SHIFT = 160, NFFT = 512, NBIN = 257, NMEL = 80;

__device__ __forceinline__ void fbank_row(const float v0, const float v1, const float pcm_scale,
                                          const float* __restrict__ window,
                                          const float* __restrict__ melw,
                                          const float* __restrict__ cmvn_mean, const float* __restrict__ cmvn_std,
                                          float* __restrict__ feat_row) {
  __shared__ float re[NFFT], im[NFFT];
  __shared__ float tw_c[NFFT / 2], tw_s[NFFT / 2];
  __shared__ float red[4];
  const int t = threadIdx.x, lane = t & 63, wave = t >> 6;
  const float x0 = v0 * pcm_scale;
  const float x1 = (t + 256 < WIN) ? v1 * pcm_scale : 0.f;
  float s = wave_sum(x0 + x1);
  if (lane == 0) red[wave] = s;
  {
    float sn, cs;
    sincospif(-2.0f * (float)t / (float)NFFT, &sn, &cs);
    tw_c[t] = cs; tw_s[t] = sn;
  }
  __syncthreads();
  const float mean = (red[0] + red[1] + red[2] + red[3]) / (float)WIN;
  re[t] = x0 - mean;
  re[t + 256] = (t + 256 < WIN) ? (x1 - mean) : 0.f;
  __syncthreads();
  float y0, y1 = 0.f;
  {
    const float prev0 = re[t > 0 ? t - 1 : 0];
    y0 = (re[t] - 0.97f * prev0) * window[t];
    if (t + 256 < WIN) y1 = (re[t + 256] - 0.97f * re[t + 255]) * window[t + 256];
  }
  __syncthreads();
  re[__brev((unsigned)t) >> 23] = y0;
  re[__brev((unsigned)(t + 256)) >> 23] = y1;
  im[t] = 0.f; im[t + 256] = 0.f;
  __syncthreads();
#pragma unroll
  for (int stg = 0; stg < 9; ++stg) {
    const int half = 1 << stg;
    const int grp = t >> stg, pos = t & (half - 1);
    const int i0 = (grp << (stg + 1)) + pos, i1 = i0 + half;
    const int tk = pos << (8 - stg);
    const float c = tw_c[tk], sn = tw_s[tk];
    const float br = re[i1] * c - im[i1] * sn;
    const float bi = re[i1] * sn + im[i1] * c;
    const float ar = re[i0], ai = im[i0];
    __syncthreads();
    re[i0] = ar + br; im[i0] = ai + bi;
    re[i1] = ar - br; im[i1] = ai - bi;
    __syncthreads();
  }
  const float p0 = re[t] * re[t] + im[t] * im[t];
  const float p256 = (t == 0) ? (re[256] * re[256] + im[256] * im[256]) : 0.f;
  __syncthreads();
  re[t] = p0;
  if (t == 0) re[256] = p256;
  __syncthreads();
  if (t < NMEL) {
    const float* w = melw + t * NBIN;
    float e = 0.f;
    for (int i = 0; i < NBIN; ++i) e = fmaf(w[i], re[i], e);
    const float lg = logf(fmaxf(e, 1.1920928955078125e-07f));
    feat_row[t] = (lg - cmvn_mean[t]) / cmvn_std[t];
  }
}

__global__ __launch_bounds__(256) void fbank_cmvn_kernel(const float* __restrict__ pcm, float pcm_scale,
                                                         const float* __restrict__ window,
                                                         const float* __restrict__ melw,
                                                         const float* __restrict__ cmvn_mean,
                                                         const float* __restrict__ cmvn_std, float* feat,
                                                         const int* __restrict__ segs,
                                                         const float* const* __restrict__ pcm_ptrs,
                                                         float* const* __restrict__ feat_ptrs) {
  const int t = threadIdx.x;
  const int frame = blockIdx.x;
  if (segs) {
    const int* sg = segs + 3 * blockIdx.y;
    if (frame >= sg[1]) return;
    if (pcm_ptrs) { pcm = pcm_ptrs[blockIdx.y]; feat = feat_ptrs[blockIdx.y]; }
    pcm += sg[0]; feat += (size_t)sg[2] * NMEL;
  }
  const float* src = pcm + (size_t)frame * SHIFT;
  fbank_row(src[t], (t + 256 < WIN) ? src[t + 256] : 0.f, pcm_scale, window, melw, cmvn_mean, cmvn_std, feat + (size_t)frame * NMEL);
}

int launch_fbank_cmvn(const float* pcm, int n_samples, float pcm_scale, const float* window,
                      const float* melw, const float* cmvn_mean, const float* cmvn_std, float* feat,
                      int* n_frames, hipStream_t stream) {
  const int T = n_samples < WIN ? 0 : 1 + (n_samples - WIN) / SHIFT;
  if (n_frames) *n_frames = T;
  if (T == 0) return SS_OK;
  hipLaunchKernelGGL(fbank_cmvn_kernel, dim3(T), dim3(256), 0, stream, pcm, pcm_scale, window, melw,
                     cmvn_mean, cmvn_std, feat, (const int*)nullptr, (const float* const*)nullptr, (float* const*)nullptr);
  SS_LAUNCH_CHECK();
  return SS_OK;
}

int launch_fbank_cmvn_batch(const float* pcm, float pcm_scale, const float* window, const float* melw,
                            const float* cmvn_mean, const float* cmvn_std, float* feat, const int* segs, int nseg,
                            int max_frames, hipStream_t stream) {
  if (nseg <= 0 || max_frames <= 0) return SS_OK;
  hipLaunchKernelGGL(fbank_cmvn_kernel, dim3(max_frames, nseg), dim3(256), 0, stream, pcm, pcm_scale, window, melw,
                     cmvn_mean, cmvn_std, feat, segs, (const float* const*)nullptr, (float* const*)nullptr);
  SS_LAUNCH_CHECK();
  return SS_OK;
}

__global__ __launch_bounds__(256) void cmvn_rows_kernel(const float* in, const float* __restrict__ cmvn_mean,
                                                        const float* __restrict__ cmvn_std, float* out, long long n) {
  const long long i = (long long)blockIdx.x * 256 + threadIdx.x;
  if (i >= n) return;
  const int t = (int)(i % NMEL);
  const float lg = in[i];
  out[i] = (lg - cmvn_mean[t]) / cmvn_std[t];
}

int launch_cmvn_rows(const float* in, long long rows, const float* cmvn_mean, const float* cmvn_std, float* out, hipStream_t stream) {
  if (rows <= 0) return SS_OK;
  const long long n = rows * NMEL, blocks = (n + 255) / 256;
  if (blocks > 0x7fffffffLL) return SS_ERR_ARG;
  hipLaunchKernelGGL(cmvn_rows_kernel, dim3((unsigned)blocks), dim3(256), 0, stream, in, cmvn_mean, cmvn_std, out, n);
  SS_LAUNCH_CHECK();
  return SS_OK;
}

int launch_fbank_cmvn_ptrs(const float* const* pcm_ptrs, float* const* feat_ptrs, float pcm_scale, const float* window,
                           const float* melw, const float* cmvn_mean, const float* cmvn_std, const int* segs, int nseg,
                           int max_frames, hipStream_t stream) {
  if (nseg <= 0 || max_frames <= 0) return SS_OK;
  hipLaunchKernelGGL(fbank_cmvn_kernel, dim3(max_frames, nseg), dim3(256), 0, stream, (const float*)nullptr, pcm_scale, window, melw,
                     cmvn_mean, cmvn_std, (float*)nullptr, segs, pcm_ptrs, feat_ptrs);
  SS_LAUNCH_CHECK();
  return SS_OK;
}

__global__ __launch_bounds__(256) void resample_kernel(const float* __restrict__ x, long long n_in, int up, int down,
                                                       const float* __restrict__ h, int half, float* __restrict__ y,
                                                       long long n_out) {
  extern __shared__ float hs[];
  const int ntaps = 2 * half + 1;
  for (int i = threadIdx.x; i < ntaps; i += 256) hs[i] = h[i];
  __syncthreads();
  const long long k = (long long)blockIdx.x * 256 + threadIdx.x;
  if (k >= n_out) return;
  y[k] = resample_sample(x, n_in, up, down, hs, half, k);
}

int launch_resample(const float* x, long long n_in, int up, int down, const float* taps, int half_len, float* y,
                    long long n_out, hipStream_t stream) {
  if (n_in <= 0 || n_out <= 0) return SS_OK;
  if (up <= 0 || down <= 0 || half_len < 0) return SS_ERR_ARG;
  const size_t lds = (size_t)(2 * half_len + 1) * sizeof(float);
  if (lds > 64 * 1024) return SS_ERR_ARG;
  hipLaunchKernelGGL(resample_kernel, dim3((unsigned)((n_out + 255) / 256)), dim3(256), lds, stream, x, n_in, up, down,
                     taps, half_len, y, n_out);
  SS_LAUNCH_CHECK();
  return SS_OK;
}

constexpr size_t FBANK_ROW_LDS = (2 * NFFT + 2 * (NFFT / 2) + 4) * sizeof(float);
constexpr size_t WG_LDS = 64 * 1024;
constexpr int FBANK_SR_MAX_HALF = (int)(((WG_LDS - FBANK_ROW_LDS) / sizeof(float) - 1) / 2);

__global__ __launch_bounds__(256) void fbank_cmvn_sr_kernel(const FbankSrSeg* __restrict__ segs, float pcm_scale,
                                                            const float* __restrict__ window, const float* __restrict__ melw,
                                                            const float* __restrict__ cmvn_mean,
                                                            const float* __restrict__ cmvn_std) {
  extern __shared__ float hs[];
  const FbankSrSeg sg = segs[blockIdx.y];
  if ((int)blockIdx.x >= sg.n_rows) return;
  const int t = threadIdx.x;
  const long long k0 = (long long)(sg.first + (int)blockIdx.x) * SHIFT + t;
  float v0, v1 = 0.f;
  if (sg.up == sg.down) {
    v0 = sg.pcm[k0];
    if (t + 256 < WIN) v1 = sg.pcm[k0 + 256];
  } else {
    const int ntaps = 2 * sg.half + 1;
    for (int i = t; i < ntaps; i += 256) hs[i] = sg.taps[i];
    __syncthreads();
    v0 = resample_sample(sg.pcm, sg.n_in, sg.up, sg.down, hs, sg.half, k0);
    if (t + 256 < WIN) v1 = resample_sample(sg.pcm, sg.n_in, sg.up, sg.down, hs, sg.half, k0 + 256);
  }
  fbank_row(v0, v1, pcm_scale, window, melw, cmvn_mean, cmvn_std, sg.feat + (size_t)blockIdx.x * NMEL);
}

int fbank_sr_rows(long long n_in, int up, int down, int half_len, int* n_rows, int* n_final) {
  if (n_in < 0 || up < 1 || down < 1 || half_len < 0) return SS_ERR_ARG;
  if (half_len > FBANK_SR_MAX_HALF) return SS_ERR_ARG;
  if (n_in > (long long)0x7fffffff || n_in * up > (long long)0x7fffffff * down) return SS_ERR_ARG;
  const long long n16 = (n_in * up + down - 1) / down;
  const long long rows = n16 < WIN ? 0 : 1 + (n16 - WIN) / SHIFT;
  const long long top = n_in * up - 1 - half_len;
  long long fin = 0;
  if (top >= 0) {
    const long long kmax = top / down;
    if (kmax >= WIN - 1) fin = 1 + (kmax - (WIN - 1)) / SHIFT;
  }
  if (fin > rows) fin = rows;
  if (n_rows) *n_rows = (int)rows;
  if (n_final) *n_final = (int)fin;
  return SS_OK;
}

int launch_fbank_cmvn_sr(const FbankSrSeg* segs, int nseg, int max_rows, int max_taps, float pcm_scale, const float* window,
                         const float* melw, const float* cmvn_mean, const float* cmvn_std, hipStream_t stream) {
  if (nseg <= 0 || max_rows <= 0) return SS_OK;
  if (max_taps < 0 || max_taps > 2 * FBANK_SR_MAX_HALF + 1) return SS_ERR_ARG;
  const size_t lds = (size_t)max_taps * sizeof(float);
  hipLaunchKernelGGL(fbank_cmvn_sr_kernel, dim3(max_rows, nseg), dim3(256), lds, stream, segs, pcm_scale, window, melw, cmvn_mean,
                     cmvn_std);
  SS_LAUNCH_CHECK();
  return SS_OK;
}

}
```

### streamspeech_amd/csrc/fbank.hpp

```cpp
#pragma once
#include <math.h>

#include "common.hpp"

namespace ss {

int launch_fbank_cmvn(const float* pcm, int n_samples, float pcm_scale, const float* window,
                      const float* melw, const float* cmvn_mean, const float* cmvn_std, float* feat,
                      int* n_frames, hipStream_t stream);

int launch_fbank_cmvn_batch(const float* pcm, float pcm_scale, const float* window, const float* melw,
                            const float* cmvn_mean, const float* cmvn_std, float* feat, const int* segs, int nseg,
                            int max_frames, hipStream_t stream);

int launch_fbank_cmvn_ptrs(const float* const* pcm_ptrs, float* const* feat_ptrs, float pcm_scale, const float* window,
                           const float* melw, const float* cmvn_mean, const float* cmvn_std, const int* segs, int nseg,
                           int max_frames, hipStream_t stream);

int launch_cmvn_rows(const float* in, long long rows, const float* cmvn_mean, const float* cmvn_std, float* out, hipStream_t stream);

int launch_resample(const float* x, long long n_in, int up, int down, const float* taps, int half_len, float* y,
                    long long n_out, hipStream_t stream);

template <class X>
__host__ __device__ __forceinline__ float resample_sample(X x, long long n_in, int up, int down, const float* hs, int half,
                                                          long long k) {
  const long long c = k * down;
  long long m_lo = c - half;
  m_lo = m_lo <= 0 ? 0 : (m_lo + up - 1) / up;
  long long m_hi = (c + half) / up;
  if (m_hi > n_in - 1) m_hi = n_in - 1;
  float acc = 0.f;
  for (long long m = m_lo; m <= m_hi; ++m) acc = fmaf(x[m], hs[half + (int)(c - m * up)], acc);
  return acc;
}

struct FbankSrSeg {
  const float* pcm;
  const float* taps;
  float* feat;
  int n_in, up, down, half, first, n_rows;
};

int fbank_sr_rows(long long n_in, int up, int down, int half_len, int* n_rows, int* n_final);

int launch_fbank_cmvn_sr(const FbankSrSeg* segs, int nseg, int max_rows, int max_taps, float pcm_scale, const float* window,
                         const float* melw, const float* cmvn_mean, const float* cmvn_std, hipStream_t stream);

}
```

### streamspeech_amd/csrc/model.hip

```cpp
#include "model_internal.hpp"

static int load_dec_layers(ss_model* m, std::vector<DecLayer>& v, const std::string& pfx, int n, int D, int F,
                           int kv_in, bool cross) {
  WeightTable& w = m->wt;
  v.resize(n);
  for (int l = 0; l < n; ++l) {
    const std::string p = pfx + ".L" + std::to_string(l) + ".";
    DecLayer& d = v[l];
    d.has_cross = cross;
    d.self_ln = {w.get(p + "self.ln.g", D), w.get(p + "self.ln.b", D)};
    d.self_qkv = {w.get(p + "self.qkv.w", 3LL * D * D), w.get(p + "self.qkv.b", 3LL * D)};
    d.self_out = {w.get(p + "self.out.w", (int64_t)D * D), w.get(p + "self.out.b", D)};
    if (cross) {
      d.cross_ln = {w.get(p + "cross.ln.g", D), w.get(p + "cross.ln.b", D)};
      d.cross_q = {w.get(p + "cross.q.w", (int64_t)D * D), w.get(p + "cross.q.b", D)};
      d.cross_kv = {w.get(p + "cross.kv.w", 2LL * D * kv_in), w.get(p + "cross.kv.b", 2LL * D)};
      d.cross_out = {w.get(p + "cross.out.w", (int64_t)D * D), w.get(p + "cross.out.b", D)};
    }
    d.ffn_ln = {w.get(p + "ffn.ln.g", D), w.get(p + "ffn.ln.b", D)};
    d.fc1 = {w.get(p + "fc1.w", (int64_t)F * D), w.get(p + "fc1.b", F)};
    d.fc2 = {w.get(p + "fc2.w", (int64_t)D * F), w.get(p + "fc2.b", D)};
  }
  return SS_OK;
}

namespace {
struct PosShared { DevBuf buf; int refs = 0; };
struct PosKey {
  int dev; const float* table; const float* w; int rows, cols;
  bool operator<(const PosKey& o) const { return std::tie(dev, table, w, rows, cols) < std::tie(o.dev, o.table, o.w, o.rows, o.cols); }
};
std::mutex g_pos_mu;
std::map<PosKey, PosShared> g_pos;
}

extern "C" int ss_abi_version(void) { return SS_ABI_VERSION; }

extern "C" const char* ss_error_string(int code) {
  switch (code) {
    case SS_OK: return "ok";
    case SS_ERR_HIP: return "HIP runtime error";
    case SS_ERR_ARG: return "invalid argument";
    case SS_ERR_MISSING_WEIGHT: return "weight slot missing or wrong size";
    case SS_ERR_CAPACITY: return "output capacity too small";
    case SS_ERR_SCRATCH_CAP: return "scratch set would grow past its cap (ss_scratch_set_cap)";
    case SS_ERR_BITSTREAM: return "corrupt or truncated MP3 bitstream";
    case SS_ERR_UNSUPPORTED: return "unsupported MP3 feature (intensity stereo, free format, Layer I/II or reserved header field)";
    case SS_ERR_STREAM_REPEAT: return "the previous streaming-encoder call timed out and its status was not checked: repeat the call";
    default: return "unknown error";
  }
}

extern "C" int ss_model_create(const ss_config* cfg, const float* d_blob, size_t blob_floats,
                               const char* const* names, const int64_t* offsets, const int64_t* numels,
                               int n_slots, ss_model** out) {
  if (!cfg || !d_blob || !out) return SS_ERR_ARG;
  if (cfg->enc_dim / cfg->enc_heads != 64 || cfg->dec_dim / cfg->dec_heads != 64) return SS_ERR_ARG;
  ss_model* m = new ss_model();
  m->cfg = *cfg;
  m->sc = new ss_scratch();
  SkScope sk_scope(m->sc->skws);
  int rc = m->wt.build(d_blob, blob_floats, names, offsets, numels, n_slots);
  if (rc != SS_OK) { ss_model_destroy(m); return rc; }
  WeightTable& w = m->wt;
  const int d = cfg->enc_dim, f = cfg->enc_ffn, D = cfg->dec_dim, F = cfg->dec_ffn, k = cfg->conv_kernel;
  const int Tm = cfg->max_rel_pos;
  m->sub0 = {w.get("enc.sub0.w", (int64_t)cfg->conv_channels * k * cfg->input_feat), w.get("enc.sub0.b", cfg->conv_channels)};
  m->sub1 = {w.get("enc.sub1.w", (int64_t)2 * d * k * (cfg->conv_channels / 2)), w.get("enc.sub1.b", 2 * d)};
  m->enc_linear = {w.get("enc.linear.w", (int64_t)d * d), w.get("enc.linear.b", d)};
  m->pos_table = w.get("enc.pos_table", (int64_t)(2 * Tm - 1) * d);
  m->pos_w = w.get("enc.pos_w", (int64_t)cfg->enc_layers * d * d);
  m->enc.resize(cfg->enc_layers);
  for (int l = 0; l < cfg->enc_layers; ++l) {
    const std::string p = "enc.L" + std::to_string(l) + ".";
    EncLayer& e = m->enc[l];
    e.ffn1_ln = {w.get(p + "ffn1.ln.g", d), w.get(p + "ffn1.ln.b", d)};
    e.ffn1_w1 = {w.get(p + "ffn1.w1.w", (int64_t)f * d), w.get(p + "ffn1.w1.b", f)};
    e.ffn1_w2 = {w.get(p + "ffn1.w2.w", (int64_t)d * f), w.get(p + "ffn1.w2.b", d)};
    e.attn_ln = {w.get(p + "attn.ln.g", d), w.get(p + "attn.ln.b", d)};
    e.qkv = {w.get(p + "attn.qkv.w", 3LL * d * d), w.get(p + "attn.qkv.b", 3LL * d)};
    e.out = {w.get(p + "attn.out.w", (int64_t)d * d), w.get(p + "attn.out.b", d)};
    e.u = w.get(p + "attn.u", d);
    e.v = w.get(p + "attn.v", d);
    e.conv_ln = {w.get(p + "conv.ln.g", d), w.get(p + "conv.ln.b", d)};
    e.pw1 = {w.get(p + "conv.pw1.w", 2LL * d * d), nullptr};
    e.dw_wt = w.get(p + "conv.dw.wt", (int64_t)cfg->dw_kernel * d);
    e.bn_mean = w.get(p + "conv.bn.mean", d);
    e.bn_var = w.get(p + "conv.bn.var", d);
    e.bn_g = w.get(p + "conv.bn.g", d);
    e.bn_b = w.get(p + "conv.bn.b", d);
    e.pw2 = {w.get(p + "conv.pw2.w", (int64_t)d * d), nullptr};
    e.ffn2_ln = {w.get(p + "ffn2.ln.g", d), w.get(p + "ffn2.ln.b", d)};
    e.ffn2_w1 = {w.get(p + "ffn2.w1.w", (int64_t)f * d), w.get(p + "ffn2.w1.b", f)};
    e.ffn2_w2 = {w.get(p + "ffn2.w2.w", (int64_t)d * f), w.get(p + "ffn2.w2.b", d)};
    e.final_ln = {w.get(p + "final_ln.g", d), w.get(p + "final_ln.b", d)};
  }
  m->ctc_asr = {w.get("ctc.asr.w", (int64_t)cfg->src_vocab * d), w.get("ctc.asr.b", cfg->src_vocab)};
  m->ctc_st = {w.get("ctc.st.w", (int64_t)cfg->tgt_vocab * d), w.get("ctc.st.b", cfg->tgt_vocab)};
  m->fe_window = w.get("fe.window", 400);
  m->fe_melw = w.get("fe.melw", 80 * 257);
  m->fe_mean = w.get("fe.cmvn_mean", 80);
  m->fe_std = w.get("fe.cmvn_std", 80);
  m->mt_emb = w.get("mt.emb", (int64_t)cfg->tgt_vocab * D);
  m->mt_pos = w.get("mt.pos_table", (int64_t)cfg->max_tgt_pos * D);
  m->mt_ln = {w.get("mt.ln.g", D), w.get("mt.ln.b", D)};
  load_dec_layers(m, m->mt, "mt", cfg->mt_layers, D, F, d, true);
  load_dec_layers(m, m->t2u, "t2u", cfg->t2u_layers, D, F, D, false);
  m->t2u_ln = {w.get("t2u.ln.g", D), w.get("t2u.ln.b", D)};
  load_dec_layers(m, m->unit, "unit", cfg->unit_layers, D, F, D, true);
  m->unit_ln = {w.get("unit.ln.g", D), w.get("unit.ln.b", D)};
  m->unit_out = {w.get("unit.out.w", (int64_t)cfg->unit_vocab * D), nullptr};
  m->unit_pos_row = w.get("unit.pos_row", D);
  if (!w.missing.empty()) { ss_model_destroy(m); return SS_ERR_MISSING_WEIGHT; }

  const int rows = 2 * Tm - 1, Ld = cfg->enc_layers * d;
  {
    int dev = 0;
    if (hipGetDevice(&dev) != hipSuccess) { ss_model_destroy(m); return SS_ERR_HIP; }
    std::lock_guard<std::mutex> lk(g_pos_mu);
    const PosKey key{dev, m->pos_table, m->pos_w, rows, Ld};
    PosShared& sh = g_pos[key];
    if (sh.refs == 0) {
      rc = sh.buf.ensure((size_t)rows * Ld * sizeof(float));
      if (rc == SS_OK) {
        Lin lp{m->pos_w, nullptr};
        rc = linear(nullptr, m->pos_table, d, rows, lp, Ld, d, sh.buf.f(), Ld);
      }
      if (rc == SS_OK && hipDeviceSynchronize() != hipSuccess) rc = SS_ERR_HIP;
      if (rc != SS_OK) { sh.buf.release(); g_pos.erase(key); }
    }
    if (rc == SS_OK) { ++sh.refs; m->pos_proj = sh.buf.f(); m->pos_key_dev = dev; }
  }
  if (rc == SS_OK) rc = scratch_fit_model(m->sc, *cfg);
  if (rc != SS_OK) { ss_model_destroy(m); return rc; }
  *out = m;
  return SS_OK;
}

extern "C" void ss_model_destroy(ss_model* m) {
  if (!m) return;
  if (m->pos_proj) {
    std::lock_guard<std::mutex> lk(g_pos_mu);
    for (auto it = g_pos.begin(); it != g_pos.end(); ++it)
      if (it->first.dev == m->pos_key_dev && it->second.buf.f() == m->pos_proj) {
        if (--it->second.refs == 0) { it->second.buf.release(); g_pos.erase(it); }
        break;
      }
  }
  scratch_unref(m->sc);
  delete m;
}

extern "C" int ss_scratch_create(ss_scratch** out) {
  if (!out) return SS_ERR_ARG;
  *out = new ss_scratch();
  return SS_OK;
}
extern "C" void ss_scratch_destroy(ss_scratch* sc) { scratch_unref(sc); }
extern "C" int ss_scratch_set_cap(ss_scratch* sc, size_t max_bytes) {
  if (!sc) return SS_ERR_ARG;
  sc->acct.cap = max_bytes;
  return SS_OK;
}
extern "C" size_t ss_scratch_bytes(ss_scratch* sc) { return sc ? sc->acct.used : 0; }
static int es_drop_stream(ss_scratch* sc);
extern "C" int ss_scratch_trim(ss_scratch* sc, size_t keep_bytes) {
  if (!sc) return SS_ERR_ARG;
  SS_HIP_CHECK(hipDeviceSynchronize());
  RET(es_drop_stream(sc));
  std::vector<DevBuf*> bufs = sc->trimmable();
  std::sort(bufs.begin(), bufs.end(), [](const DevBuf* a, const DevBuf* b) { return a->bytes > b->bytes; });
  for (DevBuf* b : bufs) {
    if (sc->acct.used <= keep_bytes) break;
    b->release();
  }
  sc->mt_Tp = 0; sc->mt_len = 0; sc->mt_enc = nullptr;
  if (!sc->es_qkv.p || !sc->es_glu.p || !sc->es_out.p) sc->es_cap = 0;
  sc->dbg_logits = nullptr; sc->dbg_rows = sc->dbg_cols = 0;
  return SS_OK;
}
extern "C" int ss_model_bind_scratch(ss_model* m, ss_scratch* sc) {
  if (!m || !sc) return SS_ERR_ARG;
  int rc = scratch_fit_model(sc, m->cfg);
  if (rc != SS_OK) return rc;
  if (sc != m->sc) {
    RET(es_drop_stream(m->sc));
    sc->refs.fetch_add(1);
    scratch_unref(m->sc);
    m->sc = sc;
  }
  return SS_OK;
}

extern "C" int ss_resample(void* stream, const float* d_in, int64_t n_in, int up, int down, const float* d_taps,
                           int half_len, float* d_out, int64_t n_out) {
  if (!d_in || !d_out || !d_taps) return SS_ERR_ARG;
  return launch_resample(d_in, n_in, up, down, d_taps, half_len, d_out, n_out, (hipStream_t)stream);
}

extern "C" int ss_row_max_logprob(void* stream, const float* d_logits, int rows, int vocab, int mask0, int mask1, int mask2,
                                  float* d_out) {
  if (!d_logits || !d_out || rows < 0 || vocab <= 0) return SS_ERR_ARG;
  return launch_row_max_logprob(d_logits, vocab, rows, vocab, mask0, mask1, mask2, d_out, (hipStream_t)stream);
}

extern "C" int ss_log_softmax(void* stream, const float* d_logits, int rows, int vocab, int mask0, int mask1, int as_probs,
                              float* d_out) {
  if (!d_logits || !d_out || rows < 0 || vocab <= 0) return SS_ERR_ARG;
  return launch_log_softmax(d_logits, vocab, rows, vocab, mask0, mask1, as_probs, d_out, vocab, (hipStream_t)stream);
}

extern "C" int ss_fbank_num_frames(int n) { return n < 400 ? 0 : 1 + (n - 400) / 160; }

extern "C" int ss_fbank_cmvn(ss_model* m, void* stream, const float* d_pcm, int n_samples, float pcm_scale,
                             float* d_feat, int* h_n_frames) {
  if (!m) return SS_ERR_ARG;
  return launch_fbank_cmvn(d_pcm, n_samples, pcm_scale, m->fe_window, m->fe_melw, m->fe_mean, m->fe_std,
                           d_feat, h_n_frames, (hipStream_t)stream);
}


extern "C" int ss_encoder_out_len(int T) {
  const int t1 = conv_out_len(T, 5, 2);
  return conv_out_len(t1, 5, 2);
}

extern "C" int ss_encoder_forward(ss_model* m, void* stream, const float* d_fbank, int T, int attn_chunk,
                                  int conv_chunk, float* d_enc_out) {
  if (!m || T <= 0) return SS_ERR_ARG;
  SkScope sk_scope(m->sc->skws);
  hipStream_t s = (hipStream_t)stream;
  const ss_config& c = m->cfg;
  const int d = c.enc_dim, f = c.enc_ffn, k = c.conv_kernel, Ld = c.enc_layers * d;
  const int T1 = conv_out_len(T, k, 2), T2 = conv_out_len(T1, k, 2);
  if (T2 <= 0 || T2 > c.max_rel_pos) return SS_ERR_CAPACITY;
  const int cchunk = conv_chunk_cfg(conv_chunk);
  const int achunk = attn_chunk_in(attn_chunk, T2);

  const size_t n_h1 = (size_t)T1 * (c.conv_channels / 2);
  const size_t n_x = (size_t)T2 * d, n_f = (size_t)T2 * f, n_qkv = (size_t)T2 * 3 * d;
  RET(m->sc->ws.ensure((n_h1 + 3 * n_x + n_f + n_qkv) * sizeof(float)));
  float* h1 = m->sc->ws.f();
  float* x = d_enc_out;
  float* h = h1 + n_h1;
  float* g = h + n_x;
  float* g2 = g + n_x;
  float* ff = g2 + n_x;
  float* qkv = ff + n_f;

  GemmArgs a, b;
  subsampler_args(m, d_fbank, h1, g, a, b);
  a.M = T1; a.in_len = T; a.chunk = cchunk;
  b.M = T2; b.in_len = T1; b.chunk = cchunk;
  RET(launch_conv_gemm(a, s));
  RET(launch_conv_gemm(b, s));
  RET(linear(s, g, d, T2, m->enc_linear, d, d, x, d));
  const float* P = m->pos_proj + (size_t)(c.max_rel_pos - T2) * Ld;

  for (int l = 0; l < c.enc_layers; ++l) {
    const EncLayer& e = m->enc[l];
    auto attention = [&]() -> int {
      AttnArgs at;
      at.Q = qkv; at.K = qkv + d; at.V = qkv + 2 * d; at.ldq = at.ldk = at.ldv = 3 * d;
      at.O = h; at.ldo = d; at.Tq = T2; at.Tk = T2; at.H = c.enc_heads; at.scale = 0.125f;
      at.chunk = achunk; at.P = P + (size_t)l * d; at.ldp = Ld; at.bias_u = e.u; at.bias_v = e.v;
      RET(bind_attn_split(m, at, s));
      return launch_attention(at, s);
    };
    auto dwconv = [&] {
      return launch_dwconv_bn_silu(g, d, g2, d, e.dw_wt, c.dw_kernel, e.bn_mean, e.bn_var, e.bn_g, e.bn_b, 1e-5f, T2, d, cchunk, s);
    };
    RET(enc_layer_ex(s, c, e, x, T2, h, ff, qkv, g, g2, false, false, attention, dwconv));
  }
  return SS_OK;
}



extern "C" int ss_encoder_stream_reset(ss_model* m) {
  if (!m) return SS_ERR_ARG;
  m->sc->es_final = 0; m->sc->es_achunk = -1; m->sc->es_cchunk = -1;
  m->sc->es_final_prev = 0;
  return SS_OK;
}

extern "C" int ss_encoder_stream_set_tail(ss_model* m, int unsettled_fbank_frames) {
  if (!m || unsettled_fbank_frames < 0) return SS_ERR_ARG;
  m->sc->es_tail = unsettled_fbank_frames;
  return SS_OK;
}

static int es_check(ss_scratch* sc, hipStream_t s, bool* repeat) {
  *repeat = false;
  SS_HIP_CHECK(hipStreamSynchronize(s));
  sc->es_pending = 0;
  unsigned e = sc->es_err_host ? *static_cast<volatile unsigned*>(sc->es_err_host) : 0u;
  const unsigned real = e;
  if (sc->es_inject) { e += 1u; sc->es_inject = 0; }
  if (!e) return SS_OK;
  fprintf(stderr, "streamspeech_hip: persistent encoder-layer launch timed out (its %d workgroups were not all resident); "
// ... 530 lines not shown
```

### streamspeech_amd/csrc/model_internal.hpp

```cpp
#pragma once
#include <algorithm>
#include <atomic>
#include <map>
#include <mutex>
#include <string>
#include <tuple>
#include <unordered_map>
#include <vector>

#include "../../include/streamspeech_hip.h"
#include "attention.hpp"
#include "attn_probs.hpp"
#include "common.hpp"
#include "elementwise.hpp"
#include "fbank.hpp"
#include "gemm.hpp"
#include "mt_step.hpp"
#include "enc_step.hpp"

using namespace ss;

namespace {

struct Slot { const float* p = nullptr; int64_t n = 0; };
// ... 135 lines not shown

struct ss_scratch {
  std::atomic<int> refs{1};
  ScratchAcct acct;
  SkWorkspace* skws = nullptr;
  DevBuf ws;
  DevBuf mt_cross;
  DevBuf mt_self;
  DevBuf mt_ws;
  int mt_Tp = 0;
  int mt_len = 0;
  const float* mt_enc = nullptr;
  DevBuf attn_split;
  DevBuf mt_gran;
  unsigned mt_epoch = 0;
  hipStream_t mt_last_stream = nullptr;
  int mt_inject_timeout = 0;
  int mt_persistent = g_mt_persistent_default;
  DevBuf mt_tok;
  DevBuf seg_buf;
  DevBuf bmt_self;
  DevBuf bmb_feat;
  DevBuf bmb_state;
  int32_t* mt_tok_host = nullptr;
  size_t mt_tok_host_n = 0;
  DevBuf es_qkv;
  DevBuf es_glu;
  DevBuf es_out;
  DevBuf es_step;
  unsigned es_bar = 0;
  int es_step_off = 0;
  int es_deferred = 0;
  int es_pending = 0;
  int es_final_prev = 0;
  int es_inject = 0;
  unsigned* es_err_host = nullptr;
  int es_cap = 0, es_final = 0, es_achunk = -1, es_cchunk = -1;
  int es_tail = 0;
  const float* dbg_logits = nullptr;
  int dbg_rows = 0, dbg_cols = 0;
  DevBuf v_ws, v_small, v_segs;
  ss_scratch() {
    for (DevBuf* b : all()) b->acct = &acct;
    skws = sk_workspace_new();
  }
  ~ss_scratch() {
    for (DevBuf* b : all()) b->release();
    if (mt_tok_host) (void)hipHostFree(mt_tok_host);
    if (es_err_host) (void)hipHostFree(es_err_host);
    sk_workspace_free(skws);
  }
  std::vector<DevBuf*> extra;
  std::vector<DevBuf*> all() {
    std::vector<DevBuf*> v = {&ws, &mt_cross, &mt_self, &mt_ws, &attn_split, &mt_gran, &mt_tok, &seg_buf, &bmt_self, &bmb_feat, &bmb_state, &es_qkv, &es_glu, &es_out, &es_step, &v_ws, &v_small, &v_segs};
    v.insert(v.end(), extra.begin(), extra.end());
    return v;
  }
  std::vector<DevBuf*> trimmable() { return {&ws, &mt_cross, &mt_ws, &seg_buf, &bmt_self, &bmb_feat, &bmb_state, &es_qkv, &es_glu, &es_out, &v_ws, &v_small, &v_segs}; }
};
[[maybe_unused]] static void scratch_unref(ss_scratch* sc) { if (sc && sc->refs.fetch_sub(1) == 1) delete sc; }
[[maybe_unused]] static int scratch_fit_model(ss_scratch* sc, const ss_config& c) {
  int rc = sc->mt_self.ensure((size_t)c.mt_layers * c.max_tgt_pos * 3 * c.dec_dim * sizeof(float));
  if (rc == SS_OK) rc = sc->mt_tok.ensure((size_t)c.max_tgt_pos * sizeof(int32_t));
  if (rc == SS_OK && sc->mt_tok_host_n < (size_t)c.max_tgt_pos) {
    if (sc->mt_tok_host) (void)hipHostFree(sc->mt_tok_host);
    sc->mt_tok_host = nullptr; sc->mt_tok_host_n = 0;
    if (hipHostMalloc((void**)&sc->mt_tok_host, (size_t)c.max_tgt_pos * sizeof(int32_t)) != hipSuccess) return SS_ERR_HIP;
    sc->mt_tok_host_n = (size_t)c.max_tgt_pos;
  }
  return rc;
}

struct ss_model {
  ss_config cfg;
  WeightTable wt;
  ss_scratch* sc = nullptr;
  Lin sub0, sub1, enc_linear, ctc_asr, ctc_st;
  std::vector<EncLayer> enc;
  const float* pos_table = nullptr;
  const float* pos_w = nullptr;
  const float* pos_proj = nullptr;
  int pos_key_dev = 0;
  const float *fe_window = nullptr, *fe_melw = nullptr, *fe_mean = nullptr, *fe_std = nullptr;
  const float* mt_emb = nullptr; const float* mt_pos = nullptr; LN mt_ln;
  std::vector<DecLayer> mt, t2u, unit;
  LN t2u_ln, unit_ln;
  Lin unit_out;
  const float* unit_pos_row = nullptr;
  int pack_invariant = g_pack_invariant_default;
};

[[maybe_unused]] static int bind_attn_split(ss_model* m, AttnArgs& at, hipStream_t s) {
  if (!m->sc->attn_split.p) {
    RET(m->sc->attn_split.ensure(attention_split_bytes()));
    SS_HIP_CHECK(hipMemsetAsync(m->sc->attn_split.p, 0, attention_split_bytes(), s));
    SS_HIP_CHECK(hipStreamSynchronize(s));
  }
  attention_bind_split(at, m->sc->attn_split.p);
  return SS_OK;
}

[[maybe_unused]] static int conv_out_len(int L, int k, int stride) { return (L + 2 * (k / 2) - k) / stride + 1; }

[[maybe_unused]] static int conv_chunk_cfg(int chunk) { return (chunk > 0 && chunk < 999) ? chunk : 0; }
[[maybe_unused]] static int attn_chunk_cfg(int chunk) { return (chunk > 0 && chunk < 999999) ? chunk : 0; }
[[maybe_unused]] static int attn_chunk_in(int chunk, int T2) { return (chunk > 0 && chunk < T2) ? chunk : 0; }

[[maybe_unused]] static int stream_final_rows(int T, int T1, int T2, int k, int achunk, int cchunk, int dwk, int tail) {
  if (achunk <= 0) return 0;
  auto reach = [&](int i, int half, int stride) {
    int r = i * stride + half;
    if (cchunk > 0) r = std::min(r, ((i * stride) / cchunk + 1) * cchunk - 1);
    return r;
  };
  int n = 0;
  for (int i = 0; i < T2; ++i) {
    const int a = reach(i, k / 2, 2);
    if (a > T1 - 1) break;
    if (reach(a, k / 2, 2) > T - 1 - tail) break;
    n = i + 1;
  }
  while (n > 0) {
    const int i = n - 1;
    const int e_att = (i / achunk + 1) * achunk - 1;
    const int e_conv = reach(i, dwk / 2, 1);
    if (std::max(e_att, e_conv) <= n - 1) break;
    --n;
  }
  return n;
}

struct StreamRows { int T1, T2, cchunk, achunk_cfg, achunk, r0, n, nf, mb1; };
[[maybe_unused]] static bool stream_rows(const ss_config& c, int T, int attn_chunk, int conv_chunk, int fin, int prev_achunk,
                                         int prev_cchunk, int tail, int max_rows, StreamRows& r) {
  const int k = c.conv_kernel;
  r.T1 = conv_out_len(T, k, 2); r.T2 = conv_out_len(r.T1, k, 2);
  if (r.T2 <= 0 || r.T2 > max_rows) return false;
  r.cchunk = conv_chunk_cfg(conv_chunk);
  r.achunk_cfg = attn_chunk_cfg(attn_chunk);
  r.achunk = attn_chunk_in(r.achunk_cfg, r.T2);
  if (prev_achunk != r.achunk_cfg || prev_cchunk != r.cchunk) fin = 0;
  if (fin > r.T2) fin = 0;
  r.r0 = fin; r.n = r.T2 - fin;
  r.nf = std::max(r.r0, stream_final_rows(T, r.T1, r.T2, k, r.achunk_cfg, r.cchunk, c.dw_kernel, tail));
  r.mb1 = std::min(std::max(0, 2 * r.r0 - k / 2), r.T1 - 1);
  return true;
}

[[maybe_unused]] static int dec_layer_ex(hipStream_t s, const ss_config& c, const DecLayer& L, float* x, int n, float* qkv_rows,
                        int ld_qkv, const AttnArgs& self_at, const AttnArgs* cross_at, float* h, float* q2, float* ff) {
  const int D = c.dec_dim, F = c.dec_ffn;
  RET(ln_linear(s, x, n, L.self_ln, L.self_qkv, 3 * D, D, qkv_rows, ld_qkv, h));
  RET(launch_attention(self_at, s));
  RET(linear(s, h, D, n, L.self_out, D, D, x, D, ACT_NONE, 1.f, x, D));
  if (L.has_cross && cross_at) {
    RET(ln_linear(s, x, n, L.cross_ln, L.cross_q, D, D, q2, D, h));
    RET(launch_attention(*cross_at, s));
    RET(linear(s, h, D, n, L.cross_out, D, D, x, D, ACT_NONE, 1.f, x, D));
  }
  RET(ln_linear(s, x, n, L.ffn_ln, L.fc1, F, D, ff, F, h, ACT_RELU));
  RET(linear(s, ff, F, n, L.fc2, D, F, x, D, ACT_NONE, 1.f, x, D));
  return SS_OK;
}

[[maybe_unused]] static int dec_layer(hipStream_t s, const ss_config& c, const DecLayer& L, float* x, int n, int pos0,
                     float* selfbuf, bool causal, const float* crossKV, int Tk_cross, float* h, float* q2,
                     float* ff, int self_tail_pad = 0, int cross_tail_pad = 0) {
  const int D = c.dec_dim, H = c.dec_heads;
  float* rows = selfbuf + (size_t)pos0 * 3 * D;
  AttnArgs at;
  at.Q = rows; at.ldq = 3 * D; at.K = selfbuf + D; at.V = selfbuf + 2 * D; at.ldk = at.ldv = 3 * D;
  at.O = h; at.ldo = D; at.Tq = n; at.Tk = pos0 + n; at.H = H; at.scale = 1.f; at.causal = causal ? 1 : 0;
  at.k_mask_tail = self_tail_pad;
  AttnArgs ac;
  if (L.has_cross) {
    ac.Q = q2; ac.ldq = D; ac.K = crossKV; ac.V = crossKV + D; ac.ldk = ac.ldv = 2 * D;
    ac.O = h; ac.ldo = D; ac.Tq = n; ac.Tk = Tk_cross; ac.H = H; ac.scale = 1.f; ac.k_mask_tail = cross_tail_pad;
  }
  return dec_layer_ex(s, c, L, x, n, rows, 3 * D, at, L.has_cross ? &ac : nullptr, h, q2, ff);
}

[[maybe_unused]] static void subsampler_args(const ss_model* m, const float* fbank, float* h1, float* out, GemmArgs& a, GemmArgs& b) {
  const ss_config& c = m->cfg;
  const int k = c.conv_kernel, C1 = c.conv_channels / 2;
  a.A = fbank; a.lda = c.input_feat; a.W = m->sub0.w; a.bias = m->sub0.b; a.C = h1; a.ldc = C1;
  a.N = c.conv_channels; a.Cin = c.input_feat; a.taps = k; a.stride = 2; a.pad = k / 2; a.glu = 1;
  b.A = h1; b.lda = C1; b.W = m->sub1.w; b.bias = m->sub1.b; b.C = out; b.ldc = c.enc_dim;
  b.N = 2 * c.enc_dim; b.Cin = C1; b.taps = k; b.stride = 2; b.pad = k / 2; b.glu = 1;
}

[[maybe_unused]] static int enc_ffn_half(hipStream_t s, const ss_config& c, float* x, int n, const LN& ln, const Lin& w1, const Lin& w2,
                                         const LN* fin, bool fused, bool canon, float* h, float* ff) {
  const int d = c.enc_dim, f = c.enc_ffn;
  if (fused)
    return launch_ffn_fused(x, d, x, d, ln.g, ln.b, w1.w, w1.b, w2.w, w2.b, 0.5f, fin ? fin->g : nullptr, fin ? fin->b : nullptr,
                            n, d, f, s, canon);
  RET(ln_linear(s, x, n, ln, w1, f, d, ff, f, h, ACT_SILU));
  RET(linear(s, ff, f, n, w2, d, f, x, d, ACT_NONE, 0.5f, x, d));
  return fin ? layernorm(s, x, x, *fin, n, d) : SS_OK;
}

template <typename Attention, typename DwConv>
static int enc_layer_ex(hipStream_t s, const ss_config& c, const EncLayer& e, float* x, int n, float* h, float* ff, float* qkv_rows,
                        float* glu_rows, const float* dw_rows, bool ffn_fused, bool canon, Attention&& attention, DwConv&& dwconv) {
  const int d = c.enc_dim;
  RET(enc_ffn_half(s, c, x, n, e.ffn1_ln, e.ffn1_w1, e.ffn1_w2, nullptr, ffn_fused, canon, h, ff));
  RET(ln_linear(s, x, n, e.attn_ln, e.qkv, 3 * d, d, qkv_rows, 3 * d, h));
  RET(attention());
  RET(linear(s, h, d, n, e.out, d, d, x, d, ACT_NONE, 1.f, x, d));
  RET(ln_linear(s, x, n, e.conv_ln, e.pw1, 2 * d, d, glu_rows, d, h, ACT_NONE, 1.f, 1));
  RET(dwconv());
  RET(linear(s, dw_rows, d, n, e.pw2, d, d, x, d, ACT_NONE, 1.f, x, d));
  return enc_ffn_half(s, c, x, n, e.ffn2_ln, e.ffn2_w1, e.ffn2_w2, &e.final_ln, ffn_fused, canon, h, ff);
}

int mt_prefix_pass(ss_model* m, hipStream_t s, int B, int Np, int np_max, int n_enc, const int* d_ptok, const int* d_ppos,
                   const int* d_pself, const int* d_pcross, const int* d_ptail, const int* d_pcache, int cache_rows, const float** out);

int mt_cross_kv(ss_model* m, hipStream_t s, const float* d_enc_out, int n_rows);

struct MtRowsWs {
  float *x, *h, *q2, *ff, *logits;
  static size_t floats(int rows, int D, int F, int V, size_t gap = 0) { return (size_t)rows * (3 * D + F + V) + gap; }
  MtRowsWs(float* base, int rows, int D, int F, size_t gap = 0)
      : x(base), h(x + (size_t)rows * D), q2(h + (size_t)rows * D), ff(q2 + (size_t)rows * D), logits(ff + (size_t)rows * F + gap) {}
};

struct MtRowsStep {
  int rows = 0;
  int cache_ld = 0, ci = 0;
  const int* tok = nullptr;
  const int* row_pos = nullptr;
  int row_pad = -1;
  const int* self_segs = nullptr;
  const int* cross_segs = nullptr;
  int n_enc = 0;
  const int* anc = nullptr; int anc_ld = 0, anc_slots = 0;
  float* states = nullptr; int states_ld = 0;
};
int mt_decode_rows(ss_model* m, hipStream_t s, const MtRowsWs& w, const MtRowsStep& a);

extern std::atomic<int> g_mt_timeouts;

struct ConvW { const float* w = nullptr; const float* b = nullptr; const float* ww = nullptr;
               const void* wh = nullptr; };
// ... 36 lines not shown
```

### streamspeech_amd/lib.py

```python
import ctypes as C
import os

_HERE = os.path.dirname(os.path.abspath(__file__))
LIB_PATH = os.environ.get("SS_HIP_LIB") or os.path.join(_HERE, "libstreamspeech_hip.so")


class SSConfig(C.Structure):
    _fields_ = [(n, C.c_int32) for n in (
        "input_feat", "conv_channels", "conv_kernel", "enc_dim", "enc_ffn", "enc_heads", "enc_layers",
        "dw_kernel", "src_vocab", "tgt_vocab", "mt_layers", "dec_dim", "dec_ffn", "dec_heads",
        "t2u_layers", "unit_layers", "unit_vocab", "ctc_upsample", "pad", "eos", "unk",
        "max_rel_pos", "max_tgt_pos")]


class SSVocoderConfig(C.Structure):
    _fields_ = [
        ("num_embeddings", C.c_int32), ("embedding_dim", C.c_int32), ("model_in_dim", C.c_int32),
        ("upsample_initial_channel", C.c_int32),
        ("n_up", C.c_int32), ("upsample_rates", C.c_int32 * 8), ("upsample_kernel_sizes", C.c_int32 * 8),
        ("n_res", C.c_int32), ("resblock_kernel_sizes", C.c_int32 * 4), ("resblock_dilations", (C.c_int32 * 3) * 4),
        ("dur_hidden", C.c_int32), ("dur_kernel", C.c_int32)]


_vp, _i, _f, _i64 = C.c_void_p, C.c_int, C.c_float, C.c_int64
# ... 205 lines not shown
                                        C.POINTER(_i64), C.POINTER(_i64), C.POINTER(C.c_int32)]),
    "ss_batch_fbank_cmvn": (_i, [_vp, _vp, _i, _vp, C.POINTER(_i64), C.POINTER(C.c_int32), _f, _vp, C.POINTER(C.c_int32)]),
    "ss_batch_cmvn": (_i, [_vp, _vp, _vp, _i64, _vp]),
    "ss_batch_encoder_forward": (_i, [_vp, _vp, _i, _vp, C.POINTER(C.c_int32), _i, _i, _vp, C.POINTER(C.c_int32)]),
    "ss_batch_ctc_greedy_scored": (_i, [_vp, _vp, _i, _i, _vp, C.POINTER(C.c_int32), _vp, _vp, _vp, _vp, _vp, _vp, _vp]),
    "ss_batch_ctc_greedy": (_i, [_vp, _vp, _i, _i, _vp, C.POINTER(C.c_int32), _vp, _vp, _vp, _vp]),
    "ss_batch_ctc_align": (_i, [_vp, _vp, _i, _i, _vp, C.POINTER(C.c_int32), C.POINTER(C.c_int32), C.POINTER(C.c_int32), _vp, _vp, _vp,
                                _vp, _vp]),
    "ss_ctc_align_host": (_i, [_vp, _i, _i, _i, _i, C.POINTER(C.c_int32), C.POINTER(C.c_int32), C.POINTER(C.c_int32), _vp, _vp, _vp,
                               _vp, _vp, _vp]),
    "ss_batch_mt_greedy": (_i, [_vp, _vp, _i, _vp, C.POINTER(C.c_int32), C.POINTER(C.c_int32), _i,
                                C.POINTER(C.c_int32), _i, C.POINTER(C.c_int32), _vp, _i]),
    "ss_batch_mt_beam": (_i, [_vp, _vp, _i, _i, _vp, C.POINTER(C.c_int32), C.POINTER(C.c_int32), _i, _f, _i,
                              C.POINTER(C.c_int32), _i, C.POINTER(C.c_int32), C.POINTER(_f), C.POINTER(_f), _vp, _i]),
    "ss_batch_mt_continue": (_i, [_vp, _vp, _i, _vp, C.POINTER(C.c_int32), C.POINTER(C.c_int32), C.POINTER(C.c_int32),
                                  C.POINTER(C.c_int32), _i, C.POINTER(C.c_int32), _i, C.POINTER(C.c_int32), _vp, _i,
                                  C.POINTER(C.c_int32)]),
    "ss_batch_mt_continue_plan": (_i, [_i, C.POINTER(C.c_int32), C.POINTER(C.c_int32), C.POINTER(C.c_int32),
                                       C.POINTER(C.c_int32), _i, _i, _i, _i, _i, _i, C.POINTER(C.c_int32), C.POINTER(C.c_int32),
                                       _i64, C.POINTER(_i64)]),
    "ss_batch_mt_beam_continue": (_i, [_vp, _vp, _i, _i, _vp, C.POINTER(C.c_int32), C.POINTER(C.c_int32), C.POINTER(C.c_int32),
                                       C.POINTER(C.c_int32), _i, _f, _i, C.POINTER(C.c_int32), _i, C.POINTER(C.c_int32),
                                       C.POINTER(_f), C.POINTER(_f), _vp, _i]),
    "ss_batch_mt_beam_continue_plan": (_i, [_i, _i, C.POINTER(C.c_int32), C.POINTER(C.c_int32), C.POINTER(C.c_int32),
                                            C.POINTER(C.c_int32), _i, _i, _i, _i, _i, _i, _i, C.POINTER(C.c_int32),
                                            C.POINTER(C.c_int32), _i64, C.POINTER(_i64)]),
    "ss_batch_mt_beam_opts": (_i, [_vp, _vp, _i, _i, _vp, C.POINTER(C.c_int32), C.POINTER(C.c_int32), _i, _f, _i,
                                   C.POINTER(C.c_int32), _i, C.POINTER(C.c_int32), C.POINTER(_f), C.POINTER(_f), _vp, _i,
                                   C.POINTER(SSMtSearchOpts)]),
    "ss_batch_mt_beam_continue_opts": (_i, [_vp, _vp, _i, _i, _vp, C.POINTER(C.c_int32), C.POINTER(C.c_int32), C.POINTER(C.c_int32),
                                            C.POINTER(C.c_int32), _i, _f, _i, C.POINTER(C.c_int32), _i, C.POINTER(C.c_int32),
                                            C.POINTER(_f), C.POINTER(_f), _vp, _i, C.POINTER(SSMtSearchOpts)]),
    "ss_batch_mt_beam_continue_plan_opts": (_i, [_i, _i, C.POINTER(C.c_int32), C.POINTER(C.c_int32), C.POINTER(C.c_int32),
                                                 C.POINTER(C.c_int32), _i, _i, _i, _i, _i, _i, _i, C.POINTER(C.c_int32),
                                                 C.POINTER(C.c_int32), _i64, C.POINTER(_i64), C.POINTER(SSMtSearchOpts)]),
    "ss_batch_mt_sample": (_i, [_vp, _vp, _i, _i, _vp, C.POINTER(C.c_int32), C.POINTER(C.c_int32), _i, _f, _i,
                                C.POINTER(C.c_int32), _i, C.POINTER(C.c_int32), C.POINTER(_f), C.POINTER(_f), _vp, _i,
                                C.POINTER(SSMtSearchOpts), C.POINTER(_i64), C.POINTER(SSMtSampleOpts)]),
    "ss_batch_mt_sample_continue": (_i, [_vp, _vp, _i, _i, _vp, C.POINTER(C.c_int32), C.POINTER(C.c_int32), C.POINTER(C.c_int32),
                                         C.POINTER(C.c_int32), _i, _f, _i, C.POINTER(C.c_int32), _i, C.POINTER(C.c_int32),
                                         C.POINTER(_f), C.POINTER(_f), _vp, _i, C.POINTER(SSMtSearchOpts), C.POINTER(_i64),
                                         C.POINTER(SSMtSampleOpts)]),
    "ss_batch_fbank_frames": (_i, [_vp, _vp, _i, C.POINTER(_vp), C.POINTER(C.c_int32), C.POINTER(C.c_int32), _f,
                                   C.POINTER(_vp)]),
    "ss_batch_fbank_frames_sr": (_i, [_vp, _vp, _i, C.POINTER(_vp), C.POINTER(C.c_int32), C.POINTER(C.c_int32), C.POINTER(C.c_int32),
                                      C.POINTER(_vp), C.POINTER(C.c_int32), C.POINTER(C.c_int32), C.POINTER(C.c_int32), _f,
                                      C.POINTER(_vp)]),
    "ss_fbank_sr_rows": (_i, [_i64, _i, _i, _i, C.POINTER(C.c_int32), C.POINTER(C.c_int32)]),
    "ss_batch_t2u_units": (_i, [_vp, _vp, _i, _vp, _i, C.POINTER(C.c_int32), _i, _i, _vp, _vp, _vp]),
    "ss_batch_vocoder_forward": (_i, [_vp, _vp, _i, _vp, C.POINTER(C.c_int32), _i, _vp, _vp, _i64, _vp,
                                      C.POINTER(_i64), C.POINTER(_i64)]),
    "ss_batch_t2u_units_pad": (_i, [_vp, _vp, _i, _vp, _i, C.POINTER(C.c_int32), C.POINTER(C.c_int32), _i, _i, _vp, _vp, _vp]),
    "ss_batch_mt_features": (_i, [_vp, _vp, _i, _vp, C.POINTER(C.c_int32), C.POINTER(C.c_int32), C.POINTER(C.c_int32),
                                  C.POINTER(C.c_int32), _vp, _i]),
    "ss_batch_mt_attention": (_i, [_vp, _vp, _i, _vp, C.POINTER(C.c_int32), C.POINTER(C.c_int32), C.POINTER(C.c_int32),
                                   C.POINTER(C.c_int32), _vp, _i, _vp, C.POINTER(_i64), _i64, _vp, _vp]),
    "ss_batch_mt_score": (_i, [_vp, _vp, _i, _vp, C.POINTER(C.c_int32), _i, C.POINTER(C.c_int32), C.POINTER(C.c_int32),
                               C.POINTER(C.c_int32), _vp, _i, _vp, _vp]),
    "ss_batch_vocoder_tail": (_i, [_vp, _vp, _i, _vp, C.POINTER(C.c_int32), C.POINTER(C.c_int32), C.POINTER(C.c_int32),
                                   C.POINTER(C.c_int32), _i, _vp, _i64, C.POINTER(C.c_int32), C.POINTER(C.c_int32),
                                   C.POINTER(_i64), C.POINTER(_i64)]),
    "ss_batch_unit_spans": (_i, [_vp, _vp, _i, _vp, C.POINTER(C.c_int32), C.POINTER(C.c_int32), C.POINTER(C.c_int32),
                                 C.POINTER(C.c_int32), _vp, _vp, _vp, _vp]),
    "ss_unit_spans_host": (_i, [_i, _vp, C.POINTER(C.c_int32), C.POINTER(C.c_int32), C.POINTER(C.c_int32), C.POINTER(C.c_int32), _vp,
                                _i, _i, _i, _i, _i, _vp, _vp]),
    "ss_op_unit_spans": (_i, [_vp, _i, _vp, C.POINTER(C.c_int32), C.POINTER(C.c_int32), C.POINTER(C.c_int32), C.POINTER(C.c_int32),
                              _vp, _i, _i, _i, _i, _i, _vp, _vp]),
    "ss_prof_enable": (_i, [_i]),
    "ss_prof_enable_hi": (_i, [_i]),
    "ss_prof_reset": (_i, []),
    "ss_prof_read": (_i, [_i, C.POINTER(C.c_double), C.POINTER(C.c_double), C.POINTER(_i64), C.POINTER(C.c_double)]),
    "ss_prof_totals": (_i, [_i, C.POINTER(C.c_double), C.POINTER(C.c_double), C.POINTER(_i64)]),
    "ss_prof_read_issued": (_i, [_i, C.POINTER(C.c_double)]),
    "ss_prof_shape_log": (_i, [_i]),
    "ss_prof_shape_dump": (_i, [C.c_char_p, _i]),
    "ss_prof_num_classes": (_i, []),
    "ss_prof_class_name": (C.c_char_p, [_i]),
    "ss_debug_force_tile": (_i, [_i, _i, _i]),
    "ss_op_ffn_fused": (_i, [_vp, _vp, _i, _vp, _i, _vp, _vp, _vp, _vp, _vp, _vp, _f, _vp, _vp, _i, _i, _i]),
    "ss_debug_ffn": (_i, [_i, _i, _i]),
    "ss_debug_rtlin": (_i, [_i, _i]),
    "ss_debug_rtlin_kb": (_i, [_i, _i]),
    "ss_debug_rtlin_kb_last": (_i, [C.POINTER(C.c_int32)]),
    "ss_debug_conv_c64": (_i, [_i]),
    "ss_debug_conv_c256_rows": (_i, [_i]),
    "ss_debug_conv_c32": (_i, [_i]),
    "ss_debug_conv_c16": (_i, [_i]),
    "ss_debug_enc_step_launches": (_i64, []),
    "ss_debug_scratch_audit": (_i, [_vp, C.POINTER(C.c_size_t), C.POINTER(C.c_size_t)]),
    "ss_op_ln_linear": (_i, [_vp, _vp, _i, _vp, _vp, _vp, _vp, _vp, _i, _vp, _i, _i, _i, _i, _i, _f, _i]),
    "ss_op_ln_linear_ex": (_i, [_vp, _vp, _i, _vp, _vp, _vp, _vp, _vp, _vp, _i, _vp, _i, _i, _i, _i, _i, _f, _i, _i]),
    "ss_debug_last_logits": (_i, [_vp, _vp, _vp, _i64, C.POINTER(_i), C.POINTER(_i)]),
    "ss_debug_sk_errors": (_i, []),
    "ss_debug_attention_split": (_i, [_i]),
    "ss_debug_attention_q16": (_i, [_i]),
    "ss_op_conv_gemm": (_i, [_vp, _vp, _i, _vp, _vp, _vp, _i, _vp, _i, _vp, _i, _i, _i, _i, _i, _i, _i, _i, _i, _i,
                             _i, _f, _i, _f, _f, _i]),
    "ss_op_conv_gemm_ex": (_i, [_vp, C.POINTER(SSOpConvArgs)]),
    "ss_op_conv_gemm_rows": (_i, [_vp, C.POINTER(SSOpConvArgs), _i, _vp, _vp, _i]),
    "ss_op_conv_pair": (_i, [_vp, _vp, _i, _vp, _vp, _vp, _vp, _vp, _i, _vp, _i, _f, _vp, _i, _f, _i, _i, _i, _i, _i, _f, _vp, _i]),
    "ss_op_resblock_fused": (_i, [_vp, _vp, _i, _vp, _vp, _vp, _vp, _vp, _vp, _i, _vp, _i, _f, _i, _i, _i, _f, _vp, _i]),
    "ss_debug_slab": (_i, [_i, C.c_longlong]),
    "ss_op_conv_f16": (_i, [_vp, _vp, _vp, _vp, _vp, _vp, _vp, _vp, _i, _i, _i, _i, _i, _f, _i, _f, _vp, _i]),
    "ss_op_layernorm": (_i, [_vp, _vp, _i, _vp, _i, _vp, _vp, _i, _i, _f]),
    "ss_op_attention": (_i, [_vp, _vp, _i, _vp, _i, _vp, _i, _vp, _i, _i, _i, _i, _f, _i, _i, _vp, _i, _vp, _vp]),
    "ss_op_attention_ex": (_i, [_vp, C.POINTER(SSOpAttnArgs)]),
    "ss_op_attention_probs": (_i, [_vp, C.POINTER(SSOpAttnProbsArgs)]),
    "ss_op_attention_pool": (_i, [_vp, C.POINTER(SSOpPoolAttnArgs)]),
    "ss_debug_attention_no_mfma": (_i, [_i]),
    "ss_op_dwconv_bn_silu": (_i, [_vp, _vp, _i, _vp, _i, _vp, _i, _vp, _vp, _vp, _vp, _f, _i, _i, _i]),
    "ss_op_dwconv_bn_silu_ex": (_i, [_vp, _vp, _i, _vp, _i, _vp, _i, _vp, _vp, _vp, _vp, _f, _i, _i, _i, _vp, _i, _i]),
    "ss_op_pool_dwconv": (_i, [_vp, _vp, _vp, _i, _vp, _vp, _i, _vp, _vp, _vp, _vp, _f, _i, _vp, _i, _i]),
    "ss_op_pool_gather_rows": (_i, [_vp, _vp, _vp, _vp, _i, _i, _vp, _vp, _i, _i]),
    "ss_op_pool_gather_ids": (_i, [_vp, _vp, _vp, _vp, _i, _vp, _vp, _i, _i]),
    "ss_op_pool_stack_rows": (_i, [_vp, _vp, _vp, _i, _vp, _vp, _i, _i]),
    "ss_op_masked_argmax": (_i, [_vp, _vp, _i, _i, _i, _i, _i, _i, _i, _vp, _vp, _i, _i, _vp, _i]),
    "ss_op_ctc_collapse": (_i, [_vp, _vp, _i, _i, _i, _vp, _vp, _vp, _vp, _i]),
    "ss_op_masked_argmax_lprob": (_i, [_vp, _vp, _i, _i, _i, _i, _i, _i, _vp, _vp]),
    "ss_op_mt_token_scores": (_i, [_vp, _vp, _i, _i, _i, _vp, _vp, _vp]),
    "ss_debug_mt_score_form": (_i, [_i]),
    "ss_op_ctc_collapse_spans": (_i, [_vp, _vp, _vp, _i, _i, _i, _vp, _vp, _vp, _vp, _vp, _vp, _i]),
    "ss_op_ctc_align": (_i, [_vp, _vp, _i, _i, _i, _i, C.POINTER(C.c_int32), C.POINTER(C.c_int32), C.POINTER(C.c_int32), _vp, _vp, _vp,
                             _vp, _vp, _vp]),
    "ss_op_dur_predict": (_i, [_vp, _vp, _vp, _i, _vp, _vp, _vp, _i]),
    "ss_op_repeat_rows": (_i, [_vp, _vp, _vp, _i, _i, _vp, _i, _vp, _i]),
    "ss_op_embed_tokens": (_i, [_vp, _vp, _vp, _vp, _f, _i, _vp, _i, _i, _i, _i, _i]),
    "ss_op_embed_tokens_rows": (_i, [_vp, _vp, _vp, _vp, _i, _f, _i, _vp, _vp, _i, _i, _i, _i]),
    "ss_op_upsample_add_pos": (_i, [_vp, _vp, _i, _i, _vp, _f, _vp, _i]),
    "ss_op_gather_rows": (_i, [_vp, _vp, _vp, _i, _vp, _i, _i]),
    "ss_op_scatter_rows": (_i, [_vp, _vp, _vp, _i, _vp, _i, _i, _i, _i]),
    "ss_op_conv_post_tanh": (_i, [_vp, _vp, _i, _i, _vp, _vp, _f, _vp, _vp, _i]),
    "ss_op_conv_post_tanh_crop": (_i, [_vp, _vp, _i, _vp, _vp, _f, _vp, _vp, _i, _i]),
    "ss_op_spkr_pre_add": (_i, [_vp, _vp, _vp, _i, _i, _vp, _vp, _i, _vp, _i, _i, _i, _i, _f]),
    "ss_op_beam_topk": (_i, [_vp, _vp, _i, _i, _i, _i, _i, _vp, _vp, _vp, _vp, _i, _i, _i, _f, _vp, _vp]),
    "ss_op_beam_merge": (_i, [_vp, C.POINTER(SSOpBeamState), _i, _i, _i, _i, _i, _i, _i, _i]),
    "ss_op_beam_prefix_score": (_i, [_vp, _vp, _i, _i, _vp, _i, _i, _f, _vp]),
    "ss_op_beam_prefix_chain": (_i, [_vp, _vp, _vp, _vp, _i, _i, _vp, _vp]),
    "ss_op_beam_topk_opts": (_i, [_vp, _vp, _i, _i, _i, _i, _i, _vp, _vp, _vp, _vp, _i, _i, _i, _f, _vp, _vp, _f, _i, _vp, _vp, _i, _i,
                                  _vp, _vp, _vp]),
    "ss_op_beam_merge_opts": (_i, [_vp, C.POINTER(SSOpBeamState), _i, _i, _i, _i, _i, _i, _i, _i, _f]),
    "ss_op_beam_prefix_score_opts": (_i, [_vp, _vp, _i, _i, _vp, _i, _i, _f, _vp, _f]),
    "ss_op_sample_step": (_i, [_vp, _vp, _i, _i, _i, _i, _vp, _vp, _i, _i, _i, _f, _f, _i, _vp, _vp, _i, _i, _vp, _vp, _vp, _vp,
                               C.POINTER(SSMtSampleOpts), _vp, _vp, _vp, _vp]),
    "ss_op_sample_uniform": (_i, [_vp, _i, _vp, _vp, _vp, _vp, _vp, _vp]),
}

_lib = None


SS_ERR_ARG = 2
SS_ERR_CAPACITY = 4
SS_ERR_SCRATCH_CAP = 5
SS_ERR_STREAM_REPEAT = 8


class StreamSpeechHipError(RuntimeError):

    def __init__(self, msg, code=None):
        super().__init__(msg)
        self.code = code


def load():
    global _lib
    if _lib is not None:
        return _lib
# ... 24 lines not shown
```

Measured before the change: 6446.

## Compute unit-decoder layer-0 QKV on distinct rows and sparsify mel filterbank

Result: faster. 6532, median of 6 (+1.3%).

```diff
diff --git a/include/streamspeech_hip.h b/include/streamspeech_hip.h
--- a/include/streamspeech_hip.h
+++ b/include/streamspeech_hip.h
@@ -414,6 +414,7 @@
                              const int32_t* h_down, const float* const* h_taps, const int32_t* h_half_len, const int32_t* h_first,
                              const int32_t* h_n, float pcm_scale, float* const* h_feat);
 int ss_fbank_sr_rows(int64_t n_in, int up, int down, int half_len, int32_t* h_n_rows, int32_t* h_n_final);
+int ss_fbank_mel_ranges(const float* h_melw, int rows, int cols, int32_t* h_lo_hi);
 int ss_batch_t2u_units(ss_model* m, void* stream, int B, const float* d_feats, int feat_rows,
                        const int32_t* h_n, int t2u_causal, int mask_eos, int32_t* d_raw, int32_t* d_tokens,
                        int32_t* d_counts);
@@ -476,6 +477,8 @@
 int ss_debug_rtlin(int grid, int enable);
 int ss_debug_rtlin_kb(int uw, int order);
 int ss_debug_rtlin_kb_last(int32_t out[4]);
+int ss_debug_unit_l0_distinct(int on);
+int ss_debug_fbank_dense(int dense);
 int ss_debug_conv_c64(int enable);
 int ss_debug_conv_c256_rows(int rows);
 int ss_debug_conv_c32(int enable);
diff --git a/streamspeech_amd/csrc/batch.hip b/streamspeech_amd/csrc/batch.hip
--- a/streamspeech_amd/csrc/batch.hip
+++ b/streamspeech_amd/csrc/batch.hip
@@ -29,7 +29,7 @@
     const int nb = std::min(kSlice, B - b0);
     int mx = 0;
     for (int b = b0; b < b0 + nb; ++b) mx = std::max(mx, segs[3 * (size_t)b + 1]);
-    RET(launch_fbank_cmvn_batch(d_pcm, pcm_scale, m->fe_window, m->fe_melw, m->fe_mean, m->fe_std, d_feat, dt + 3 * (size_t)b0, nb,
+    RET(launch_fbank_cmvn_batch(d_pcm, pcm_scale, m->fe_window, m->fe_melw, fe_tables(m), m->fe_mean, m->fe_std, d_feat, dt + 3 * (size_t)b0, nb,
                                 mx, s));
   }
   return SS_OK;
@@ -299,8 +299,9 @@
   const Offsets on = prefix(h_n, B);
   const int Nn = on.total, U = Nn * up;
   const size_t nx = (size_t)U * D;
+  const bool l0_distinct = m->pack_invariant && !debug_tile_forced() && disp().unit_l0_distinct && c.unit_layers > 0 && up > 1;
   RET(m->sc->ws.ensure((3 * nx + (size_t)U * 3 * D + (size_t)U * F + (size_t)Nn * 2 * D + (size_t)Nn * D +
-                    (size_t)U * V + (size_t)U) * sizeof(float)));
+                    (l0_distinct ? (size_t)Nn * 4 * D : 0) + (size_t)U * V + (size_t)U) * sizeof(float)));
   float* x = m->sc->ws.f();
   float* h = x + nx;
   float* q2 = h + nx;
@@ -308,7 +309,9 @@
   float* ff = selfbuf + (size_t)U * 3 * D;
   float* crosskv = ff + (size_t)U * F;
   float* t2u_out = crosskv + (size_t)Nn * 2 * D;
-  float* logits = t2u_out + (size_t)Nn * D;
+  float* x0 = t2u_out + (size_t)Nn * D;
+  float* qkv0 = x0 + (size_t)Nn * D;
+  float* logits = l0_distinct ? qkv0 + (size_t)Nn * 3 * D : x0;
   int32_t* idx_scratch = reinterpret_cast<int32_t*>(logits + (size_t)U * V);
   std::vector<int> tab(14 * B + Nn + (h_pad ? 3 * B : 0));
   for (int b = 0; b < B; ++b) {
@@ -352,6 +355,13 @@
     ac.O = h; ac.ldo = D; ac.H = H; ac.scale = 1.f; ac.segs = dt + 8 * B; ac.nseg = B; ac.max_q = on.mx * up;
     ac.no_decode_kernel = m->pack_invariant;
     if (tail) { at.seg_tail = tail + B; ac.seg_tail = tail + 2 * B; }
+    if (l == 0 && l0_distinct) {
+      RET(launch_upsample_add_pos(t2u_out, Nn, 1, m->unit_pos_row, (float)c.pad, x0, D, s));
+      RET(dec_layer_qkv(s, c, m->unit[0], x0, Nn, qkv0, 3 * D, h));
+      RET(launch_upsample_rows(qkv0, Nn, up, selfbuf, 3 * D, s));
+      RET(dec_layer_rest(s, c, m->unit[0], x, U, at, &ac, h, q2, ff));
+      continue;
+    }
     RET(dec_layer_ex(s, c, m->unit[l], x, U, selfbuf, 3 * D, at, &ac, h, q2, ff));
   }
   RET(launch_layernorm(x, D, h, D, m->unit_ln.g, m->unit_ln.b, U, D, 1e-5f, s));
@@ -755,7 +765,7 @@
   RET(upload(s, dt, tab));
   const float* const* d_pcm = reinterpret_cast<const float* const*>(dt + n_seg);
   float* const* d_feat = reinterpret_cast<float* const*>(dt + n_seg + 2 * (size_t)B);
-  return launch_fbank_cmvn_ptrs(d_pcm, d_feat, pcm_scale, m->fe_window, m->fe_melw, m->fe_mean, m->fe_std, dt, B, mx, s);
+  return launch_fbank_cmvn_ptrs(d_pcm, d_feat, pcm_scale, m->fe_window, m->fe_melw, fe_tables(m), m->fe_mean, m->fe_std, dt, B, mx, s);
 }
 
 extern "C" int ss_batch_fbank_frames_sr(ss_model* m, void* stream, int B, const float* const* h_pcm, const int32_t* h_n_in,
@@ -789,7 +799,7 @@
   RET(m->sc->seg_buf.ensure(tab.size() * sizeof(int)));
   int* dt = (int*)m->sc->seg_buf.p;
   RET(upload(s, dt, tab));
-  return launch_fbank_cmvn_sr(reinterpret_cast<const FbankSrSeg*>(dt), B, mx, max_taps, pcm_scale, m->fe_window, m->fe_melw,
+  return launch_fbank_cmvn_sr(reinterpret_cast<const FbankSrSeg*>(dt), B, mx, max_taps, pcm_scale, m->fe_window, m->fe_melw, fe_tables(m),
                               m->fe_mean, m->fe_std, s);
 }
 
diff --git a/streamspeech_amd/csrc/debug_ops.hip b/streamspeech_amd/csrc/debug_ops.hip
--- a/streamspeech_amd/csrc/debug_ops.hip
+++ b/streamspeech_amd/csrc/debug_ops.hip
@@ -175,6 +175,16 @@
   int v[4];
   rtlin_kb_last(v);
   for (int i = 0; i < 4; ++i) out[i] = v[i];
+  return SS_OK;
+}
+extern "C" int ss_debug_unit_l0_distinct(int on) {
+  if (on < -1 || on > 1) return SS_ERR_ARG;
+  dispatch_edit([on](Dispatch& d) { d.unit_l0_distinct = on < 0 ? (getenv("SS_UNIT_L0_DISTINCT") ? atoi(getenv("SS_UNIT_L0_DISTINCT")) != 0 : 1) : on; });
+  return SS_OK;
+}
+extern "C" int ss_debug_fbank_dense(int dense) {
+  if (dense < -1 || dense > 1) return SS_ERR_ARG;
+  dispatch_edit([dense](Dispatch& d) { d.fbank_dense = dense < 0 ? (getenv("SS_FBANK_DENSE") ? atoi(getenv("SS_FBANK_DENSE")) != 0 : 0) : dense; });
   return SS_OK;
 }
 extern "C" int ss_debug_ffn(int grid, int row_tiles_per_wave, int enable) {
diff --git a/streamspeech_amd/csrc/dispatch.hip b/streamspeech_amd/csrc/dispatch.hip
--- a/streamspeech_amd/csrc/dispatch.hip
+++ b/streamspeech_amd/csrc/dispatch.hip
@@ -33,6 +33,7 @@
   d.smallm_max_rows = I("SS_SMALLM_MAX_ROWS", d.smallm_max_rows); d.sk_min_units = L("SS_SK_MIN_UNITS", d.sk_min_units);
   d.no_sk2 = I("SS_NO_SK2", 0) ? 1 : 0; d.sk2_min_k64 = I("SS_SK2_MINK64", d.sk2_min_k64); d.sk2_spare_cus = I("SS_SK2_SPARE_CUS", 0);
   d.rt_wg_per_cu = I("SS_RTLIN_WG_PER_CU", 0); d.c32_min_k = I("SS_CONV_C32_MIN_K", d.c32_min_k); d.c16_min_k = I("SS_CONV_C16_MIN_K", d.c16_min_k);
+  d.unit_l0_distinct = I("SS_UNIT_L0_DISTINCT", 1) ? 1 : 0; d.fbank_dense = I("SS_FBANK_DENSE", 0) ? 1 : 0;
   return d;
 }
 Dispatch& process_settings() { static Dispatch d = env_defaults(); return d; }
diff --git a/streamspeech_amd/csrc/dispatch.hpp b/streamspeech_amd/csrc/dispatch.hpp
--- a/streamspeech_amd/csrc/dispatch.hpp
+++ b/streamspeech_amd/csrc/dispatch.hpp
@@ -36,6 +36,8 @@
   int rt_kb_xmap = 1;
   int rt_kb_uw = 0;
   int rt_kb_order = 1;
+  int unit_l0_distinct = 1;
+  int fbank_dense = 0;
 };
 
 const Dispatch& disp();
diff --git a/streamspeech_amd/csrc/elementwise.hip b/streamspeech_amd/csrc/elementwise.hip
--- a/streamspeech_amd/csrc/elementwise.hip
+++ b/streamspeech_amd/csrc/elementwise.hip
@@ -168,6 +168,24 @@
   if (n <= 0) return SS_OK;
   hipLaunchKernelGGL(upsample_add_pos_kernel, dim3(cdiv(D, 256), n * up), dim3(256), 0, stream, src, up,
                      pos_row, pad_value, out, D);
+  SS_LAUNCH_CHECK();
+  return SS_OK;
+}
+
+__global__ __launch_bounds__(256) void upsample_rows_kernel(const float4* __restrict__ src, int up, float4* __restrict__ out, int D4) {
+  const int u = blockIdx.x;
+  const float4* s = src + (size_t)(u / up) * D4;
+  float4* o = out + (size_t)u * D4;
+  for (int c = threadIdx.x; c < D4; c += 256) o[c] = s[c];
+}
+
+int launch_upsample_rows(const float* src, int n, int up, float* out, int D, hipStream_t stream) {
+  if (n <= 0) return SS_OK;
+  if (up <= 0 || D <= 0 || (D & 3) || (long long)n * up > 0x7fffffffLL || !src || !out ||
+      ((uintptr_t)src & 15) || ((uintptr_t)out & 15))
+    return SS_ERR_ARG;
+  hipLaunchKernelGGL(upsample_rows_kernel, dim3((unsigned)(n * up)), dim3(256), 0, stream, reinterpret_cast<const float4*>(src), up,
+                     reinterpret_cast<float4*>(out), D / 4);
   SS_LAUNCH_CHECK();
   return SS_OK;
 }
diff --git a/streamspeech_amd/csrc/elementwise.hpp b/streamspeech_amd/csrc/elementwise.hpp
--- a/streamspeech_amd/csrc/elementwise.hpp
+++ b/streamspeech_amd/csrc/elementwise.hpp
@@ -21,6 +21,8 @@
 
 int launch_upsample_add_pos(const float* src, int n, int up, const float* pos_row, float pad_value,
                             float* out, int D, hipStream_t stream);
+
+int launch_upsample_rows(const float* src, int n, int up, float* out, int D, hipStream_t stream);
 
 int launch_masked_argmax(const float* logits, int ld, int M, int N, int mask0, int mask1, int mask2,
                          int force, int* ids, hipStream_t stream, const int* row_max_len = nullptr, int step = 0,
diff --git a/streamspeech_amd/csrc/fbank.hip b/streamspeech_amd/csrc/fbank.hip
--- a/streamspeech_amd/csrc/fbank.hip
+++ b/streamspeech_amd/csrc/fbank.hip
@@ -7,6 +7,7 @@
 __device__ __forceinline__ void fbank_row(const float v0, const float v1, const float pcm_scale,
                                           const float* __restrict__ window,
                                           const float* __restrict__ melw,
+                                          const FbankTables tabs,
                                           const float* __restrict__ cmvn_mean, const float* __restrict__ cmvn_std,
                                           float* __restrict__ feat_row) {
   __shared__ float re[NFFT], im[NFFT];
@@ -17,7 +18,9 @@
   const float x1 = (t + 256 < WIN) ? v1 * pcm_scale : 0.f;
   float s = wave_sum(x0 + x1);
   if (lane == 0) red[wave] = s;
-  {
+  if (tabs.twiddle) {
+    tw_c[t] = tabs.twiddle[t]; tw_s[t] = tabs.twiddle[NFFT / 2 + t];
+  } else {
     float sn, cs;
     sincospif(-2.0f * (float)t / (float)NFFT, &sn, &cs);
     tw_c[t] = cs; tw_s[t] = sn;
@@ -61,8 +64,12 @@
   __syncthreads();
   if (t < NMEL) {
     const float* w = melw + t * NBIN;
+    int lo = 0, hi = NBIN;
+    if (tabs.mel_range) {
+      lo = max(tabs.mel_range[2 * t], 0); hi = min(tabs.mel_range[2 * t + 1], NBIN);
+    }
     float e = 0.f;
-    for (int i = 0; i < NBIN; ++i) e = fmaf(w[i], re[i], e);
+    for (int i = lo; i < hi; ++i) e = fmaf(w[i], re[i], e);
     const float lg = logf(fmaxf(e, 1.1920928955078125e-07f));
     feat_row[t] = (lg - cmvn_mean[t]) / cmvn_std[t];
   }
@@ -71,6 +78,7 @@
 __global__ __launch_bounds__(256) void fbank_cmvn_kernel(const float* __restrict__ pcm, float pcm_scale,
                                                          const float* __restrict__ window,
                                                          const float* __restrict__ melw,
+                                                         const FbankTables tabs,
                                                          const float* __restrict__ cmvn_mean,
                                                          const float* __restrict__ cmvn_std, float* feat,
                                                          const int* __restrict__ segs,
@@ -85,27 +93,53 @@
     pcm += sg[0]; feat += (size_t)sg[2] * NMEL;
   }
   const float* src = pcm + (size_t)frame * SHIFT;
-  fbank_row(src[t], (t + 256 < WIN) ? src[t + 256] : 0.f, pcm_scale, window, melw, cmvn_mean, cmvn_std, feat + (size_t)frame * NMEL);
+  fbank_row(src[t], (t + 256 < WIN) ? src[t + 256] : 0.f, pcm_scale, window, melw, tabs, cmvn_mean, cmvn_std, feat + (size_t)frame * NMEL);
+}
+
+__global__ __launch_bounds__(256) void fbank_twiddle_kernel(float* __restrict__ tw) {
+  const int t = threadIdx.x;
+  float sn, cs;
+  sincospif(-2.0f * (float)t / (float)NFFT, &sn, &cs);
+  tw[t] = cs; tw[NFFT / 2 + t] = sn;
+}
+
+int launch_fbank_twiddles(float* tw, hipStream_t stream) {
+  if (!tw) return SS_ERR_ARG;
+  hipLaunchKernelGGL(fbank_twiddle_kernel, dim3(1), dim3(NFFT / 2), 0, stream, tw);
+  SS_LAUNCH_CHECK();
+  return SS_OK;
+}
+
+int fbank_mel_ranges(const float* melw, int rows, int cols, int* lo_hi) {
+  if (!melw || !lo_hi || rows < 0 || cols < 0) return SS_ERR_ARG;
+  for (int r = 0; r < rows; ++r) {
+    const float* w = melw + (size_t)r * cols;
+    int lo = 0, hi = 0;
+    for (int i = 0; i < cols; ++i)
+      if (w[i] != 0.f) { if (hi == 0) lo = i; hi = i + 1; }
+    lo_hi[2 * r] = lo; lo_hi[2 * r + 1] = hi;
+  }
+  return SS_OK;
 }
 
 int launch_fbank_cmvn(const float* pcm, int n_samples, float pcm_scale, const float* window,
-                      const float* melw, const float* cmvn_mean, const float* cmvn_std, float* feat,
+                      const float* melw, const FbankTables& tabs, const float* cmvn_mean, const float* cmvn_std, float* feat,
                       int* n_frames, hipStream_t stream) {
   const int T = n_samples < WIN ? 0 : 1 + (n_samples - WIN) / SHIFT;
   if (n_frames) *n_frames = T;
   if (T == 0) return SS_OK;
   hipLaunchKernelGGL(fbank_cmvn_kernel, dim3(T), dim3(256), 0, stream, pcm, pcm_scale, window, melw,
-                     cmvn_mean, cmvn_std, feat, (const int*)nullptr, (const float* const*)nullptr, (float* const*)nullptr);
+                     tabs, cmvn_mean, cmvn_std, feat, (const int*)nullptr, (const float* const*)nullptr, (float* const*)nullptr);
   SS_LAUNCH_CHECK();
   return SS_OK;
 }
 
 int launch_fbank_cmvn_batch(const float* pcm, float pcm_scale, const float* window, const float* melw,
-                            const float* cmvn_mean, const float* cmvn_std, float* feat, const int* segs, int nseg,
+                            const FbankTables& tabs, const float* cmvn_mean, const float* cmvn_std, float* feat, const int* segs, int nseg,
                             int max_frames, hipStream_t stream) {
   if (nseg <= 0 || max_frames <= 0) return SS_OK;
   hipLaunchKernelGGL(fbank_cmvn_kernel, dim3(max_frames, nseg), dim3(256), 0, stream, pcm, pcm_scale, window, melw,
-                     cmvn_mean, cmvn_std, feat, segs, (const float* const*)nullptr, (float* const*)nullptr);
+                     tabs, cmvn_mean, cmvn_std, feat, segs, (const float* const*)nullptr, (float* const*)nullptr);
   SS_LAUNCH_CHECK();
   return SS_OK;
 }
@@ -129,11 +163,11 @@
 }
 
 int launch_fbank_cmvn_ptrs(const float* const* pcm_ptrs, float* const* feat_ptrs, float pcm_scale, const float* window,
-                           const float* melw, const float* cmvn_mean, const float* cmvn_std, const int* segs, int nseg,
-                           int max_frames, hipStream_t stream) {
+                           const float* melw, const FbankTables& tabs, const float* cmvn_mean, const float* cmvn_std,
+                           const int* segs, int nseg, int max_frames, hipStream_t stream) {
   if (nseg <= 0 || max_frames <= 0) return SS_OK;
   hipLaunchKernelGGL(fbank_cmvn_kernel, dim3(max_frames, nseg), dim3(256), 0, stream, (const float*)nullptr, pcm_scale, window, melw,
-                     cmvn_mean, cmvn_std, (float*)nullptr, segs, pcm_ptrs, feat_ptrs);
+                     tabs, cmvn_mean, cmvn_std, (float*)nullptr, segs, pcm_ptrs, feat_ptrs);
   SS_LAUNCH_CHECK();
   return SS_OK;
 }
@@ -168,7 +202,7 @@
 
 __global__ __launch_bounds__(256) void fbank_cmvn_sr_kernel(const FbankSrSeg* __restrict__ segs, float pcm_scale,
                                                             const float* __restrict__ window, const float* __restrict__ melw,
-                                                            const float* __restrict__ cmvn_mean,
+                                                            const FbankTables tabs, const float* __restrict__ cmvn_mean,
                                                             const float* __restrict__ cmvn_std) {
   extern __shared__ float hs[];
   const FbankSrSeg sg = segs[blockIdx.y];
@@ -186,7 +220,7 @@
     v0 = resample_sample(sg.pcm, sg.n_in, sg.up, sg.down, hs, sg.half, k0);
     if (t + 256 < WIN) v1 = resample_sample(sg.pcm, sg.n_in, sg.up, sg.down, hs, sg.half, k0 + 256);
   }
-  fbank_row(v0, v1, pcm_scale, window, melw, cmvn_mean, cmvn_std, sg.feat + (size_t)blockIdx.x * NMEL);
+  fbank_row(v0, v1, pcm_scale, window, melw, tabs, cmvn_mean, cmvn_std, sg.feat + (size_t)blockIdx.x * NMEL);
 }
 
 int fbank_sr_rows(long long n_in, int up, int down, int half_len, int* n_rows, int* n_final) {
@@ -208,14 +242,15 @@
 }
 
 int launch_fbank_cmvn_sr(const FbankSrSeg* segs, int nseg, int max_rows, int max_taps, float pcm_scale, const float* window,
-                         const float* melw, const float* cmvn_mean, const float* cmvn_std, hipStream_t stream) {
+                         const float* melw, const FbankTables& tabs, const float* cmvn_mean, const float* cmvn_std,
+                         hipStream_t stream) {
   if (nseg <= 0 || max_rows <= 0) return SS_OK;
   if (max_taps < 0 || max_taps > 2 * FBANK_SR_MAX_HALF + 1) return SS_ERR_ARG;
   const size_t lds = (size_t)max_taps * sizeof(float);
-  hipLaunchKernelGGL(fbank_cmvn_sr_kernel, dim3(max_rows, nseg), dim3(256), lds, stream, segs, pcm_scale, window, melw, cmvn_mean,
-                     cmvn_std);
-  SS_LAUNCH_CHECK();
-  return SS_OK;
-}
-
-}
+  hipLaunchKernelGGL(fbank_cmvn_sr_kernel, dim3(max_rows, nseg), dim3(256), lds, stream, segs, pcm_scale, window, melw, tabs,
+                     cmvn_mean, cmvn_std);
+  SS_LAUNCH_CHECK();
+  return SS_OK;
+}
+
+}
diff --git a/streamspeech_amd/csrc/fbank.hpp b/streamspeech_amd/csrc/fbank.hpp
--- a/streamspeech_amd/csrc/fbank.hpp
+++ b/streamspeech_amd/csrc/fbank.hpp
@@ -5,17 +5,25 @@
 
 namespace ss {
 
+struct FbankTables {
+  const int* mel_range = nullptr;
+  const float* twiddle = nullptr;
+};
+
+int fbank_mel_ranges(const float* melw, int rows, int cols, int* lo_hi);
+int launch_fbank_twiddles(float* tw, hipStream_t stream);
+
 int launch_fbank_cmvn(const float* pcm, int n_samples, float pcm_scale, const float* window,
-                      const float* melw, const float* cmvn_mean, const float* cmvn_std, float* feat,
+                      const float* melw, const FbankTables& tabs, const float* cmvn_mean, const float* cmvn_std, float* feat,
                       int* n_frames, hipStream_t stream);
 
 int launch_fbank_cmvn_batch(const float* pcm, float pcm_scale, const float* window, const float* melw,
-                            const float* cmvn_mean, const float* cmvn_std, float* feat, const int* segs, int nseg,
+                            const FbankTables& tabs, const float* cmvn_mean, const float* cmvn_std, float* feat, const int* segs, int nseg,
                             int max_frames, hipStream_t stream);
 
 int launch_fbank_cmvn_ptrs(const float* const* pcm_ptrs, float* const* feat_ptrs, float pcm_scale, const float* window,
-                           const float* melw, const float* cmvn_mean, const float* cmvn_std, const int* segs, int nseg,
-                           int max_frames, hipStream_t stream);
+                           const float* melw, const FbankTables& tabs, const float* cmvn_mean, const float* cmvn_std,
+                           const int* segs, int nseg, int max_frames, hipStream_t stream);
 
 int launch_cmvn_rows(const float* in, long long rows, const float* cmvn_mean, const float* cmvn_std, float* out, hipStream_t stream);
 
@@ -45,6 +53,7 @@
 int fbank_sr_rows(long long n_in, int up, int down, int half_len, int* n_rows, int* n_final);
 
 int launch_fbank_cmvn_sr(const FbankSrSeg* segs, int nseg, int max_rows, int max_taps, float pcm_scale, const float* window,
-                         const float* melw, const float* cmvn_mean, const float* cmvn_std, hipStream_t stream);
+                         const float* melw, const FbankTables& tabs, const float* cmvn_mean, const float* cmvn_std,
+                         hipStream_t stream);
 
 }
diff --git a/streamspeech_amd/csrc/model.hip b/streamspeech_amd/csrc/model.hip
--- a/streamspeech_amd/csrc/model.hip
+++ b/streamspeech_amd/csrc/model.hip
@@ -49,6 +49,27 @@
     case SS_ERR_STREAM_REPEAT: return "the previous streaming-encoder call timed out and its status was not checked: repeat the call";
     default: return "unknown error";
   }
+}
+
+static int make_fbank_tables(ss_model* m) {
+  constexpr int R = 80, Cn = 257, NTW = 512;
+  std::vector<float> melw((size_t)R * Cn);
+  SS_HIP_CHECK(hipMemcpy(melw.data(), m->fe_melw, melw.size() * sizeof(float), hipMemcpyDeviceToHost));
+  std::vector<int> rng(2 * R);
+  RET(fbank_mel_ranges(melw.data(), R, Cn, rng.data()));
+  RET(m->fe_tab.ensure(rng.size() * sizeof(int) + NTW * sizeof(float), true));
+  int* d_rng = reinterpret_cast<int*>(m->fe_tab.p);
+  float* d_tw = reinterpret_cast<float*>(d_rng + rng.size());
+  SS_HIP_CHECK(hipMemcpy(d_rng, rng.data(), rng.size() * sizeof(int), hipMemcpyHostToDevice));
+  RET(launch_fbank_twiddles(d_tw, nullptr));
+  SS_HIP_CHECK(hipDeviceSynchronize());
+  m->fe_tables.mel_range = d_rng;
+  m->fe_tables.twiddle = d_tw;
+  return SS_OK;
+}
+
+extern "C" int ss_fbank_mel_ranges(const float* h_melw, int rows, int cols, int32_t* h_lo_hi) {
+  return fbank_mel_ranges(h_melw, rows, cols, h_lo_hi);
 }
 
 extern "C" int ss_model_create(const ss_config* cfg, const float* d_blob, size_t blob_floats,
@@ -112,6 +133,8 @@
   m->unit_out = {w.get("unit.out.w", (int64_t)cfg->unit_vocab * D), nullptr};
   m->unit_pos_row = w.get("unit.pos_row", D);
   if (!w.missing.empty()) { ss_model_destroy(m); return SS_ERR_MISSING_WEIGHT; }
+  rc = make_fbank_tables(m);
+  if (rc != SS_OK) { ss_model_destroy(m); return rc; }
 
   const int rows = 2 * Tm - 1, Ld = cfg->enc_layers * d;
   {
@@ -147,6 +170,7 @@
         break;
       }
   }
+  m->fe_tab.release();
   scratch_unref(m->sc);
   delete m;
 }
@@ -215,7 +239,7 @@
 extern "C" int ss_fbank_cmvn(ss_model* m, void* stream, const float* d_pcm, int n_samples, float pcm_scale,
                              float* d_feat, int* h_n_frames) {
   if (!m) return SS_ERR_ARG;
-  return launch_fbank_cmvn(d_pcm, n_samples, pcm_scale, m->fe_window, m->fe_melw, m->fe_mean, m->fe_std,
+  return launch_fbank_cmvn(d_pcm, n_samples, pcm_scale, m->fe_window, m->fe_melw, fe_tables(m), m->fe_mean, m->fe_std,
                            d_feat, h_n_frames, (hipStream_t)stream);
 }
 
diff --git a/streamspeech_amd/csrc/model_internal.hpp b/streamspeech_amd/csrc/model_internal.hpp
--- a/streamspeech_amd/csrc/model_internal.hpp
+++ b/streamspeech_amd/csrc/model_internal.hpp
@@ -241,6 +241,8 @@
   const float* pos_proj = nullptr;
   int pos_key_dev = 0;
   const float *fe_window = nullptr, *fe_melw = nullptr, *fe_mean = nullptr, *fe_std = nullptr;
+  DevBuf fe_tab;
+  FbankTables fe_tables;
   const float* mt_emb = nullptr; const float* mt_pos = nullptr; LN mt_ln;
   std::vector<DecLayer> mt, t2u, unit;
   LN t2u_ln, unit_ln;
@@ -248,6 +250,8 @@
   const float* unit_pos_row = nullptr;
   int pack_invariant = g_pack_invariant_default;
 };
+
+[[maybe_unused]] static FbankTables fe_tables(const ss_model* m) { return disp().fbank_dense ? FbankTables{} : m->fe_tables; }
 
 [[maybe_unused]] static int bind_attn_split(ss_model* m, AttnArgs& at, hipStream_t s) {
   if (!m->sc->attn_split.p) {
@@ -306,10 +310,14 @@
   return true;
 }
 
-[[maybe_unused]] static int dec_layer_ex(hipStream_t s, const ss_config& c, const DecLayer& L, float* x, int n, float* qkv_rows,
-                        int ld_qkv, const AttnArgs& self_at, const AttnArgs* cross_at, float* h, float* q2, float* ff) {
+[[maybe_unused]] static int dec_layer_qkv(hipStream_t s, const ss_config& c, const DecLayer& L, const float* x, int n, float* qkv_rows,
+                         int ld_qkv, float* h) {
+  const int D = c.dec_dim;
+  return ln_linear(s, x, n, L.self_ln, L.self_qkv, 3 * D, D, qkv_rows, ld_qkv, h);
+}
+[[maybe_unused]] static int dec_layer_rest(hipStream_t s, const ss_config& c, const DecLayer& L, float* x, int n, const AttnArgs& self_at,
+                          const AttnArgs* cross_at, float* h, float* q2, float* ff) {
   const int D = c.dec_dim, F = c.dec_ffn;
-  RET(ln_linear(s, x, n, L.self_ln, L.self_qkv, 3 * D, D, qkv_rows, ld_qkv, h));
   RET(launch_attention(self_at, s));
   RET(linear(s, h, D, n, L.self_out, D, D, x, D, ACT_NONE, 1.f, x, D));
   if (L.has_cross && cross_at) {
@@ -320,6 +328,11 @@
   RET(ln_linear(s, x, n, L.ffn_ln, L.fc1, F, D, ff, F, h, ACT_RELU));
   RET(linear(s, ff, F, n, L.fc2, D, F, x, D, ACT_NONE, 1.f, x, D));
   return SS_OK;
+}
+[[maybe_unused]] static int dec_layer_ex(hipStream_t s, const ss_config& c, const DecLayer& L, float* x, int n, float* qkv_rows,
+                        int ld_qkv, const AttnArgs& self_at, const AttnArgs* cross_at, float* h, float* q2, float* ff) {
+  RET(dec_layer_qkv(s, c, L, x, n, qkv_rows, ld_qkv, h));
+  return dec_layer_rest(s, c, L, x, n, self_at, cross_at, h, q2, ff);
 }
 
 [[maybe_unused]] static int dec_layer(hipStream_t s, const ss_config& c, const DecLayer& L, float* x, int n, int pos0,
diff --git a/streamspeech_amd/lib.py b/streamspeech_amd/lib.py
--- a/streamspeech_amd/lib.py
+++ b/streamspeech_amd/lib.py
@@ -311,6 +311,9 @@
     "ss_debug_rtlin": (_i, [_i, _i]),
     "ss_debug_rtlin_kb": (_i, [_i, _i]),
     "ss_debug_rtlin_kb_last": (_i, [C.POINTER(C.c_int32)]),
+    "ss_debug_unit_l0_distinct": (_i, [_i]),
+    "ss_debug_fbank_dense": (_i, [_i]),
+    "ss_fbank_mel_ranges": (_i, [_vp, _i, _i, C.POINTER(C.c_int32)]),
     "ss_debug_conv_c64": (_i, [_i]),
     "ss_debug_conv_c256_rows": (_i, [_i]),
     "ss_debug_conv_c32": (_i, [_i]),
```
